# xuekt98/BBDM

Hardware: NVIDIA H100
Metric: denoising-steps/sec (UNet fwd) at 256^2 pixel-BBDM (higher is better)
Workload: dtype bf16x3 (split-bf16 tensor-core products, fp32 accumulate: fp32-class)

## Files before the change

bbdm_b200/cabi.py:

```python
from __future__ import annotations

import ctypes as C
import gc
import os

import torch

_HERE = os.path.dirname(os.path.abspath(__file__))
LIB_PATH = os.environ.get("BBDM_LIB") or os.path.join(_HERE, "libbbdm_b200.so")

ABI_VERSION = 7
OBJ = {"grad": 0, "noise": 1, "ysubx": 2}
RESAMPLE_NONE, RESAMPLE_UP2, RESAMPLE_DOWN2 = 0, 1, 2
RES_NONE, RES_SAME, RES_UP2, RES_DOWN2 = 0, 1, 2, 3
GN_MAX_SLICES = 64
ATTN_HEAD_DIMS = (16, 32, 64, 128)
ATTN_TC_HEAD_DIMS = (64, 128)
LN_MAX_C = 2048


def layernorm_bwd_workspace(rows, C):
    return -(-rows // 64) * 2 * C

SYMBOLS = [
    "bbdm_abi_version", "bbdm_last_error", "bbdm_device_info", "bbdm_check_device_fault",
    "bbdm_bridge_q_sample", "bbdm_bridge_p_sample", "bbdm_bridge_p_sample_dev", "bbdm_nchw_to_nhwc_cat", "bbdm_nhwc_to_nchw",
    "bbdm_gather_rows", "bbdm_linear_f32", "bbdm_gn_stats", "bbdm_prep_operand",
    "bbdm_pack_weight_split", "bbdm_pack_weight_split_padded", "bbdm_pack_weight_split_taps", "bbdm_pack_weight_split_dgrad",
    "bbdm_pack_weight_f32", "bbdm_conv_umma", "bbdm_conv_direct",
    "bbdm_attention", "bbdm_attention_split", "bbdm_attention_tc", "bbdm_conv_umma_geometry", "bbdm_gn_finalize_partials",
    "bbdm_split_grad", "bbdm_conv_wgrad_workspace", "bbdm_conv_wgrad", "bbdm_gn_bwd_reduce", "bbdm_gn_bwd_apply",
    "bbdm_conv_wgrad_direct", "bbdm_attention_bwd", "bbdm_conv_direct_pad", "bbdm_softmax_rows_split", "bbdm_vq_nearest", "bbdm_s2d_split", "bbdm_pack_weight_split_both",
    "bbdm_wino_geometry", "bbdm_wino_input", "bbdm_wino_output", "bbdm_wino_pack_weight",
    "bbdm_wino6_geometry", "bbdm_wino6_input", "bbdm_wino6_output", "bbdm_wino6_pack_weight",
    "bbdm_optim_chunk_elems", "bbdm_adam_multi", "bbdm_ema_multi", "bbdm_denorm_to_uint8",
    "bbdm_layernorm_split", "bbdm_geglu_split", "bbdm_attention_cross", "bbdm_conv_stem", "bbdm_spatial_rescale",
    "bbdm_layernorm_bwd", "bbdm_geglu_bwd", "bbdm_attention_cross_bwd",
]


class PSampleCoef(C.Structure):
    _fields_ = [("m_t", C.c_float), ("one_minus_m_t", C.c_float), ("sqrt_var_t", C.c_float),
                ("m_nt", C.c_float), ("one_minus_m_nt", C.c_float), ("c_xt", C.c_float),
                ("sigma_t", C.c_float)]


class PrepArgs(C.Structure):
    _fields_ = [("src1", C.c_void_p), ("c1", C.c_int), ("src2", C.c_void_p), ("c2", C.c_int),
                ("B", C.c_int), ("Hs", C.c_int), ("Ws", C.c_int), ("groups", C.c_int),
                ("mean", C.c_void_p), ("rstd", C.c_void_p), ("gamma", C.c_void_p), ("beta", C.c_void_p),
                ("film_scale", C.c_void_p), ("film_shift", C.c_void_p), ("film_stride", C.c_int64),
                ("silu", C.c_int), ("resample", C.c_int),
                ("act_f32", C.c_void_p), ("act_hi", C.c_void_p), ("act_lo", C.c_void_p),
                ("raw_f32", C.c_void_p), ("raw_hi", C.c_void_p), ("raw_lo", C.c_void_p)]


class ConvArgs(C.Structure):
    _fields_ = [("B", C.c_int), ("H", C.c_int), ("W", C.c_int),
                ("Cin", C.c_int), ("Cout", C.c_int), ("taps", C.c_int),
                ("a_hi", C.c_void_p), ("a_lo", C.c_void_p), ("w_hi", C.c_void_p), ("w_lo", C.c_void_p),
                ("bias", C.c_void_p),
                ("Cin2", C.c_int),
                ("a2_hi", C.c_void_p), ("a2_lo", C.c_void_p), ("w2_hi", C.c_void_p), ("w2_lo", C.c_void_p),
                ("bias2", C.c_void_p),
                ("residual", C.c_void_p), ("res_mode", C.c_int),
                ("out", C.c_void_p), ("out_hi", C.c_void_p), ("out_lo", C.c_void_p),
                ("passes", C.c_int), ("out_nchw_channels", C.c_int), ("upsample2x", C.c_int),
                ("stats_partial", C.c_void_p), ("weights_per_image", C.c_int), ("operand_f16", C.c_int),
                ("window_origin", C.c_int)]


class WinoInputArgs(C.Structure):
    _fields_ = [("src1", C.c_void_p), ("c1", C.c_int), ("src2", C.c_void_p), ("c2", C.c_int),
                ("B", C.c_int), ("H", C.c_int), ("W", C.c_int), ("groups", C.c_int),
                ("mean", C.c_void_p), ("rstd", C.c_void_p), ("gamma", C.c_void_p), ("beta", C.c_void_p),
                ("film_scale", C.c_void_p), ("film_shift", C.c_void_p), ("film_stride", C.c_int64),
                ("silu", C.c_int),
                ("v_hi", C.c_void_p), ("v_lo", C.c_void_p), ("raw_hi", C.c_void_p), ("raw_lo", C.c_void_p),
                ("act_hi", C.c_void_p), ("act_lo", C.c_void_p), ("down2", C.c_int)]


class WinoOutputArgs(C.Structure):
    _fields_ = [("m", C.c_void_p), ("inv_wscale", C.c_void_p), ("B", C.c_int), ("H", C.c_int), ("W", C.c_int), ("Cout", C.c_int),
                ("bias", C.c_void_p), ("residual", C.c_void_p), ("res_mode", C.c_int),
                ("out", C.c_void_p), ("stats_partial", C.c_void_p), ("up2_phases", C.c_int)]


class BbdmError(RuntimeError):
    pass


_lib = None


def load():
    global _lib
    if _lib is not None:
        return _lib
    if not os.path.exists(LIB_PATH):
        raise BbdmError(
            f"{LIB_PATH} not found: build the sm_90a kernels first (python -m bbdm_b200.build). "
            "bbdm_b200 has no PyTorch/CPU fallback for its kernels.")
    lib = C.CDLL(LIB_PATH)
    vp, i, i64, f = C.c_void_p, C.c_int, C.c_int64, C.c_float
    lib.bbdm_abi_version.restype = i
    lib.bbdm_last_error.restype = C.c_char_p
    lib.bbdm_device_info.argtypes = [C.POINTER(i)] * 3
    lib.bbdm_check_device_fault.argtypes = [vp, C.POINTER(C.c_ulonglong)]
    lib.bbdm_bridge_q_sample.argtypes = [vp, vp, vp, vp, vp, vp, i, i, vp, vp, i, i64, vp]
    lib.bbdm_bridge_p_sample.argtypes = [vp, vp, vp, vp, PSampleCoef, i, i, i, vp, vp, i64, vp]
    lib.bbdm_bridge_p_sample_dev.argtypes = [vp, vp, vp, vp, vp, i, i, i, vp, vp, i64, vp]
    lib.bbdm_nchw_to_nhwc_cat.argtypes = [vp, i, vp, i, i, i, i, vp, vp]
    lib.bbdm_nhwc_to_nchw.argtypes = [vp, i, i, i, i, vp, vp]
    lib.bbdm_gather_rows.argtypes = [vp, i, i, vp, i, vp, vp]
    lib.bbdm_linear_f32.argtypes = [vp, vp, vp, vp, i, i, i, i, i, vp]
    lib.bbdm_gn_stats.argtypes = [vp, i, vp, i, i, i, i, i, f, vp, vp, vp, vp]
    lib.bbdm_prep_operand.argtypes = [C.POINTER(PrepArgs), vp]
    lib.bbdm_pack_weight_split.argtypes = [vp, i, i, i, vp, vp, vp]
    lib.bbdm_pack_weight_split_padded.argtypes = [vp, i, i, i, i, vp, vp, vp]
    lib.bbdm_pack_weight_split_dgrad.argtypes = [vp, i, i, i, vp, vp, vp]
    lib.bbdm_pack_weight_split_taps.argtypes = [vp, i, i, i, vp, vp, vp]
    lib.bbdm_pack_weight_f32.argtypes = [vp, i, i, i, vp, vp]
    lib.bbdm_conv_umma.argtypes = [C.POINTER(ConvArgs), vp]
    lib.bbdm_conv_direct.argtypes = [vp, vp, vp, vp, vp, i, i, i, i, i, i, i, vp]
    lib.bbdm_conv_stem.argtypes = [vp, vp, vp, vp, i, i, i, i, i, vp, vp]
    lib.bbdm_attention.argtypes = [vp, i, i, i, i, i, vp, vp, vp, vp]
    lib.bbdm_conv_umma_geometry.argtypes = [i, i, C.POINTER(i), C.POINTER(i), C.POINTER(i), C.POINTER(i)]
    lib.bbdm_gn_finalize_partials.argtypes = [vp, i, i, vp, i, i, i, i, i, f, vp, vp, vp]
    lib.bbdm_split_grad.argtypes = [vp, i64, i, vp, vp, vp, vp, i64, vp, vp, vp]
    lib.bbdm_conv_wgrad_workspace.argtypes = [i, i, i, i, i, i, C.POINTER(i), C.POINTER(i64)]
    lib.bbdm_conv_wgrad.argtypes = [vp, vp, i64, vp, vp, i, i, i, i, i, i, i, vp, vp, vp]
    lib.bbdm_conv_wgrad_direct.argtypes = [vp, vp, i, i, i, i, i, i, vp, vp, i64, vp]
    lib.bbdm_gn_bwd_reduce.argtypes = [vp, vp, i, i, i, i, i, vp, vp, vp, vp, vp, vp, i64, i, vp, vp, vp]
    lib.bbdm_gn_bwd_apply.argtypes = [vp, vp, i, i, i, i, i, vp, vp, vp, vp, vp, vp, i64, i, vp, vp, vp, vp]
    lib.bbdm_attention_split.argtypes = [vp, vp, i, i, i, i, i, vp, vp, vp, vp]
    lib.bbdm_attention_tc.argtypes = [vp, vp, i, i, i, i, i, vp, vp, vp, vp]
    lib.bbdm_attention_bwd.argtypes = [vp, vp, vp, i, i, i, i, i, vp, vp, vp, vp]
    lib.bbdm_conv_direct_pad.argtypes = [vp, vp, vp, vp, vp, i, i, i, i, i, i, i, i, i, vp]
    lib.bbdm_softmax_rows_split.argtypes = [vp, i64, i64, C.c_float, vp, vp, vp]
    lib.bbdm_vq_nearest.argtypes = [vp, vp, i64, i, i, vp, vp, vp]
    lib.bbdm_s2d_split.argtypes = [vp, i, i, i, i, vp, vp, vp]
    lib.bbdm_pack_weight_split_both.argtypes = [vp, i, i, i, vp, vp, vp, vp, vp]
    lib.bbdm_wino_geometry.argtypes = [i, i, i, C.POINTER(i), C.POINTER(i), C.POINTER(i64), C.POINTER(i)]
    lib.bbdm_wino_input.argtypes = [C.POINTER(WinoInputArgs), vp]
    lib.bbdm_wino_output.argtypes = [C.POINTER(WinoOutputArgs), vp]
    lib.bbdm_wino_pack_weight.argtypes = [vp, i, i, i, vp, vp, vp, vp]
    lib.bbdm_wino6_geometry.argtypes = lib.bbdm_wino_geometry.argtypes
    lib.bbdm_wino6_input.argtypes = lib.bbdm_wino_input.argtypes
    lib.bbdm_wino6_output.argtypes = lib.bbdm_wino_output.argtypes
    lib.bbdm_wino6_pack_weight.argtypes = lib.bbdm_wino_pack_weight.argtypes
    lib.bbdm_denorm_to_uint8.argtypes = [vp, i, i, i, i, i, vp, vp]
    lib.bbdm_spatial_rescale.argtypes = [vp, i, i, i, i, i, vp, vp, i, vp, vp]
    lib.bbdm_layernorm_split.argtypes = [vp, i64, i, vp, vp, f, vp, vp, vp, vp]
    lib.bbdm_geglu_split.argtypes = [vp, i64, i, vp, vp, vp, vp]
    lib.bbdm_attention_cross.argtypes = [vp, vp, vp, vp, i, i, i, i, i, vp, vp, vp, vp]
    lib.bbdm_layernorm_bwd.argtypes = [vp, vp, i64, i, vp, f, vp, vp, vp, vp, vp]
    lib.bbdm_geglu_bwd.argtypes = [vp, vp, i64, i, vp, vp]
    lib.bbdm_attention_cross_bwd.argtypes = [vp, vp, vp, vp, i, i, i, i, i, vp, vp, vp, vp, vp]
    lib.bbdm_optim_chunk_elems.argtypes = []
    lib.bbdm_adam_multi.argtypes = [vp, vp, vp, vp, vp, vp, i, vp, vp, C.c_double, C.c_double, C.c_double, C.c_double,
                                     C.c_double, i64, vp, C.c_double, vp]
    lib.bbdm_ema_multi.argtypes = [vp, vp, vp, vp, vp, i, vp, C.c_double, i, vp]
    for s in SYMBOLS:
        fn = getattr(lib, s)
        if s not in ("bbdm_last_error",):
            fn.restype = i
    if lib.bbdm_abi_version() != ABI_VERSION:
        raise BbdmError(f"libbbdm_b200.so ABI {lib.bbdm_abi_version()} != binding ABI {ABI_VERSION}")
    _lib = lib
    return lib


def check(rc: int):
    if rc != 0:
        raise BbdmError(f"bbdm_b200 C-ABI call failed ({rc}): {load().bbdm_last_error().decode()}")


def ptr(t):
    return None if t is None else t.data_ptr()


def stream():
    return torch.cuda.current_stream().cuda_stream


def _device_guarded(fn):
    import functools

    @functools.wraps(fn)
    def wrapper(self, *args, **kw):
        dev = None
        for a in args:
            if isinstance(a, torch.Tensor) and a.is_cuda:
                dev = a.device.index
                break
        if dev is None:
            for a in kw.values():
                if isinstance(a, torch.Tensor) and a.is_cuda:
                    dev = a.device.index
                    break
        if dev is None or dev == torch.cuda.current_device():
            return fn(self, *args, **kw)
        with torch.cuda.device(dev):
            return fn(self, *args, **kw)
    return wrapper


def _guard_all(cls):
    for name, fn in list(vars(cls).items()):
        if callable(fn) and not name.startswith("_") and name not in ("empty", "conv_geometry", "wgrad_workspace", "wino_geometry", "optim_chunk_elems"):
            setattr(cls, name, _device_guarded(fn))
    return cls


LAUNCHES = {"n": 0}


def _req(t, dtype=torch.float32):
    assert t.is_cuda and t.is_contiguous() and t.dtype == dtype, (t.device, t.dtype, t.is_contiguous())
    return t


def _pitch(hi_t, lo_t, rows, cols):
    assert hi_t.is_cuda and tuple(hi_t.shape) == (rows, cols) and hi_t.stride(1) == 1, (hi_t.shape, hi_t.stride())
    assert lo_t.shape == hi_t.shape and lo_t.stride() == hi_t.stride(), (hi_t.stride(), lo_t.stride())
    return hi_t.stride(0)


@_guard_all
class CudaBackend:

    name = "sm_90a"
    requires_cuda = True
    wino_tensor_scale = True
    wino_tiles = (4, 6)
    window_origin = True

    def __init__(self):
        self.lib = load()

    def empty(self, shape, dtype, device):
        try:
            return torch.empty(shape, dtype=dtype, device=device)
        except torch.OutOfMemoryError:
            gc.collect()
            return torch.empty(shape, dtype=dtype, device=device)

    def q_sample(self, x0, y, noise, t, m_t, var_t, objective, xt_out, obj_out):
        B = x0.shape[0]
        n = x0.numel() // B
        for z in (x0, y, noise, m_t, var_t, xt_out, obj_out):
            _req(z)
        _req(t, torch.int64)
        check(self.lib.bbdm_bridge_q_sample(ptr(x0), ptr(y), ptr(noise), ptr(t), ptr(m_t), ptr(var_t),
                                            m_t.numel(), OBJ[objective], ptr(xt_out), ptr(obj_out), B, n,
                                            stream()))
        LAUNCHES["n"] += 1

    def p_sample(self, x_t, y, eps, noise, coef, objective, clip, is_last, x_out, x0_out):
        for z in (x_t, y, eps, x_out):
            _req(z)
        c = PSampleCoef(*[float(v) for v in coef])
        check(self.lib.bbdm_bridge_p_sample(ptr(x_t), ptr(y), ptr(eps), ptr(noise), c, OBJ[objective],
                                            int(clip), int(is_last), ptr(x_out), ptr(x0_out), x_t.numel(),
                                            stream()))
        LAUNCHES["n"] += 1

    def p_sample_dev(self, x_t, y, eps, noise, coef_dev, objective, clip, is_last, x_out, x0_out):
        for z in (x_t, y, eps, x_out, coef_dev):
            _req(z)
        check(self.lib.bbdm_bridge_p_sample_dev(ptr(x_t), ptr(y), ptr(eps), ptr(noise), ptr(coef_dev),
                                                OBJ[objective], int(clip), int(is_last), ptr(x_out), ptr(x0_out),
                                                x_t.numel(), stream()))
        LAUNCHES["n"] += 1

    def nchw_to_nhwc_cat(self, x, ctx, out):
        B, c1, H, W = x.shape
        c2 = 0 if ctx is None else ctx.shape[1]
        check(self.lib.bbdm_nchw_to_nhwc_cat(ptr(_req(x)), c1, ptr(ctx), c2, B, H, W, ptr(_req(out)), stream()))
        LAUNCHES["n"] += 1

    def nhwc_to_nchw(self, src, out):
        B, H, W, Cc = src.shape
        check(self.lib.bbdm_nhwc_to_nchw(ptr(_req(src)), B, H, W, Cc, ptr(_req(out)), stream()))
        LAUNCHES["n"] += 1

    def gather_rows(self, table, idx, out):
        check(self.lib.bbdm_gather_rows(ptr(_req(table)), table.shape[0], table.shape[1],
                                        ptr(_req(idx, torch.int64)), idx.numel(), ptr(_req(out)), stream()))
        LAUNCHES["n"] += 1

    def linear(self, x, w, bias, out, act_in=False, act_out=False):
        B, K = x.shape
        N = w.shape[0]
        check(self.lib.bbdm_linear_f32(ptr(_req(x)), ptr(_req(w)), ptr(bias), ptr(_req(out)), B, K, N,
                                       int(act_in), int(act_out), stream()))
        LAUNCHES["n"] += (B + 7) // 8

    def gn_stats(self, src1, src2, groups, eps, mean, rstd, workspace):
        B, H, W, c1 = src1.shape
        c2 = 0 if src2 is None else src2.shape[3]
        check(self.lib.bbdm_gn_stats(ptr(_req(src1)), c1, ptr(src2), c2, B, H, W, groups, eps,
                                     ptr(_req(mean)), ptr(_req(rstd)), ptr(workspace), stream()))
        LAUNCHES["n"] += 2

    def prep(self, src1, src2, *, groups=32, mean=None, rstd=None, gamma=None, beta=None,
             film_scale=None, film_shift=None, film_stride=0, silu=True, resample=RESAMPLE_NONE,
             act_f32=None, act_hi=None, act_lo=None, raw_f32=None, raw_hi=None, raw_lo=None):
        B, Hs, Ws, c1 = src1.shape
        a = PrepArgs(ptr(_req(src1)), c1, ptr(src2), 0 if src2 is None else src2.shape[3], B, Hs, Ws, groups,
                     ptr(mean), ptr(rstd), ptr(gamma), ptr(beta), ptr(film_scale), ptr(film_shift),
                     film_stride, int(silu), resample, ptr(act_f32), ptr(act_hi), ptr(act_lo),
                     ptr(raw_f32), ptr(raw_hi), ptr(raw_lo))
        check(self.lib.bbdm_prep_operand(C.byref(a), stream()))
        LAUNCHES["n"] += 1

    def pack_weight_split(self, w, hi, lo):
        Cout, Cin, k = w.shape[0], w.shape[1], (w.shape[2] if w.dim() > 2 else 1)
        check(self.lib.bbdm_pack_weight_split_padded(ptr(_req(w)), Cout, Cin, k, hi.shape[1], ptr(hi), ptr(lo),
                                                     stream()))
        LAUNCHES["n"] += 1

    def pack_weight_split_dgrad(self, w, hi, lo):
        Cout, Cin, k = w.shape[0], w.shape[1], w.shape[2]
        check(self.lib.bbdm_pack_weight_split_dgrad(ptr(_req(w)), Cout, Cin, k, ptr(hi), ptr(lo), stream()))
        LAUNCHES["n"] += 1

    def pack_weight_split_both(self, w, f_hi, f_lo, d_hi=None, d_lo=None):
        Cout, Cin, k = w.shape[0], w.shape[1], w.shape[2]
        check(self.lib.bbdm_pack_weight_split_both(ptr(_req(w)), Cout, Cin, k, ptr(f_hi), ptr(f_lo), ptr(d_hi), ptr(d_lo),
                                                   stream()))
        LAUNCHES["n"] += 1

    def pack_weight_split_taps(self, w, hi, lo):
        Cout, Cin, taps = w.shape
        check(self.lib.bbdm_pack_weight_split_taps(ptr(_req(w)), Cout, Cin, taps, ptr(hi), ptr(lo), stream()))
        LAUNCHES["n"] += 1

    def pack_weight_f32(self, w, out):
        Cout, Cin, k = w.shape[0], w.shape[1], (w.shape[2] if w.dim() > 2 else 1)
        check(self.lib.bbdm_pack_weight_f32(ptr(_req(w)), Cout, Cin, k, ptr(_req(out)), stream()))
        LAUNCHES["n"] += 1

    def conv_umma(self, *, B, H, W, Cin, Cout, taps, a_hi, a_lo, w_hi, w_lo, bias=None, Cin2=0,
                  a2_hi=None, a2_lo=None, w2_hi=None, w2_lo=None, bias2=None, residual=None,
                  res_mode=RES_NONE, out=None, out_hi=None, out_lo=None, passes=3, out_nchw_channels=0,
                  stats_partial=None, upsample2x=False, weights_per_image=False, operand_f16=False, window_origin=0):
        a = ConvArgs(B, H, W, Cin, Cout, taps, ptr(a_hi), ptr(a_lo), ptr(w_hi), ptr(w_lo), ptr(bias),
                     Cin2, ptr(a2_hi), ptr(a2_lo), ptr(w2_hi), ptr(w2_lo), ptr(bias2),
                     ptr(residual), res_mode, ptr(out), ptr(out_hi), ptr(out_lo), passes, out_nchw_channels,
                     int(upsample2x), ptr(stats_partial), int(weights_per_image), int(operand_f16), int(window_origin))
        check(self.lib.bbdm_conv_umma(C.byref(a), stream()))
        LAUNCHES["n"] += 1

    def conv_geometry(self, H, W):
        v = [C.c_int(0) for _ in range(4)]
        check(self.lib.bbdm_conv_umma_geometry(H, W, *[C.byref(z) for z in v]))
        return tuple(z.value for z in v)

    def _wino(self, name, tile):
        assert tile in self.wino_tiles, tile
        return getattr(self.lib, f"bbdm_wino{'' if tile == 4 else tile}_{name}")

    def wino_geometry(self, B, H, W, tile=4):
        th, tw, el, tot = C.c_int(0), C.c_int(0), C.c_int(0), C.c_int64(0)
        check(self._wino("geometry", tile)(B, H, W, C.byref(th), C.byref(tw), C.byref(tot), C.byref(el)))
        return th.value, tw.value, tot.value, bool(el.value)

    def wino_input(self, src1, src2, *, groups=32, mean=None, rstd=None, gamma=None, beta=None, film_scale=None,
                   film_shift=None, film_stride=0, silu=True, v_hi, v_lo, raw_hi=None, raw_lo=None, act_hi=None,
                   act_lo=None, tile=4, down2=False):
        B, H, W, c1 = src1.shape
        a = WinoInputArgs(ptr(_req(src1)), c1, ptr(src2), 0 if src2 is None else src2.shape[3], B, H, W, groups,
                          ptr(mean), ptr(rstd), ptr(gamma), ptr(beta), ptr(film_scale), ptr(film_shift), film_stride,
                          int(silu), ptr(_req(v_hi, torch.float16)), ptr(_req(v_lo, torch.float16)),
                          ptr(raw_hi), ptr(raw_lo), ptr(act_hi), ptr(act_lo), int(down2))
        check(self._wino("input", tile)(C.byref(a), stream()))
        LAUNCHES["n"] += 1

    def wino_output(self, m, *, B, H, W, Cout, bias=None, residual=None, res_mode=RES_NONE, out, stats_partial=None,
                    inv_wscale=None, tile=4, up2_phases=False):
        a = WinoOutputArgs(ptr(_req(m)), None if inv_wscale is None else ptr(_req(inv_wscale)), B, H, W, Cout, ptr(bias), ptr(residual), res_mode, ptr(_req(out)),
                           ptr(stats_partial), int(up2_phases))
        check(self._wino("output", tile)(C.byref(a), stream()))
        LAUNCHES["n"] += 1

    def wino_pack_weight(self, w, u_hi, u_lo, dgrad=False, inv_wscale=None, tile=4):
        Cout, Cin = w.shape[0], w.shape[1]
        check(self._wino("pack_weight", tile)(ptr(_req(w)), Cout, Cin, int(dgrad), ptr(_req(u_hi, torch.float16)),
                                              ptr(_req(u_lo, torch.float16)),
                                              None if inv_wscale is None else ptr(_req(inv_wscale)), stream()))
        LAUNCHES["n"] += 1

    def layernorm_split(self, x, gamma, beta, eps, out_f32=None, out_hi=None, out_lo=None):
        Cc = x.shape[-1]
        check(self.lib.bbdm_layernorm_split(ptr(_req(x)), x.numel() // Cc, Cc, ptr(_req(gamma)), ptr(_req(beta)), eps,
                                            ptr(out_f32), ptr(out_hi), ptr(out_lo), stream()))
        LAUNCHES["n"] += 1

    def geglu_split(self, u, out_f32=None, out_hi=None, out_lo=None):
        N2 = u.shape[-1]
        check(self.lib.bbdm_geglu_split(ptr(_req(u)), u.numel() // N2, N2 // 2, ptr(out_f32), ptr(out_hi), ptr(out_lo),
                                        stream()))
        LAUNCHES["n"] += 1

    def attention_cross(self, q_hi, q_lo, kv_hi, kv_lo, heads, out_f32=None, out_hi=None, out_lo=None):
        B, Tq, Cc = q_hi.shape
        Tkv = kv_hi.shape[1]
        check(self.lib.bbdm_attention_cross(ptr(_req(q_hi, torch.bfloat16)), ptr(_req(q_lo, torch.bfloat16)),
                                            ptr(_req(kv_hi, torch.bfloat16)), ptr(_req(kv_lo, torch.bfloat16)), B, Tq, Tkv,
                                            Cc, heads, ptr(out_f32), ptr(out_hi), ptr(out_lo), stream()))
        LAUNCHES["n"] += 1

    def layernorm_bwd(self, x, dy, gamma, eps, dx, dgamma, dbeta, workspace):
        Cc = x.shape[-1]
        check(self.lib.bbdm_layernorm_bwd(ptr(_req(x)), ptr(_req(dy)), x.numel() // Cc, Cc, ptr(_req(gamma)), eps,
                                          ptr(_req(dx)), ptr(_req(dgamma)), ptr(_req(dbeta)), ptr(_req(workspace)),
                                          stream()))
        LAUNCHES["n"] += 2

    def geglu_bwd(self, u, dy, du):
        N2 = u.shape[-1]
        check(self.lib.bbdm_geglu_bwd(ptr(_req(u)), ptr(_req(dy)), u.numel() // N2, N2 // 2, ptr(_req(du)), stream()))
        LAUNCHES["n"] += 1

    def attention_cross_bwd(self, q, kv, out, dout, heads, dq, dkv, lse, delta):
        B, Tq, Cc = q.shape
        check(self.lib.bbdm_attention_cross_bwd(ptr(_req(q)), ptr(_req(kv)), ptr(_req(out)), ptr(_req(dout)), B, Tq,
                                                kv.shape[1], Cc, heads, ptr(_req(dq)), ptr(_req(dkv)), ptr(_req(lse)),
                                                ptr(_req(delta)), stream()))
        LAUNCHES["n"] += 2

    def denorm_to_uint8(self, images, to_normal, out):
        B, Cc, H, W = images.shape
        check(self.lib.bbdm_denorm_to_uint8(ptr(_req(images)), B, Cc, H, W, int(to_normal), ptr(_req(out, torch.uint8)),
                                            stream()))
        LAUNCHES["n"] += 1

    def spatial_rescale(self, src, n_stages, weight, bias, out):
        B, Cc, H, W = src.shape
        cout = 0 if weight is None else int(weight.shape[0])
        check(self.lib.bbdm_spatial_rescale(ptr(_req(src)), B, Cc, H, W, int(n_stages),
                                            ptr(None if weight is None else _req(weight)),
                                            ptr(None if bias is None else _req(bias)), cout, ptr(_req(out)), stream()))
        LAUNCHES["n"] += 1

    def optim_chunk_elems(self):
        return int(self.lib.bbdm_optim_chunk_elems())

    def adam_multi(self, tab, exp_avg, exp_avg_sq, *, lr, beta1, beta2, eps, weight_decay, step, ema_shadow=None,
                   ema_decay=0.0):
        check(self.lib.bbdm_adam_multi(ptr(tab.params), ptr(tab.grads), ptr(tab.numel), ptr(tab.offsets),
                                       ptr(tab.chunk_tensor), ptr(tab.chunk_index), tab.n_chunks, ptr(_req(exp_avg)),
                                       ptr(_req(exp_avg_sq)), lr, beta1, beta2, eps, weight_decay, int(step),
                                       ptr(ema_shadow), float(ema_decay), stream()))
        LAUNCHES["n"] += 1

    def ema_multi(self, tab, shadow, decay, with_decay=True):
        check(self.lib.bbdm_ema_multi(ptr(tab.params), ptr(tab.numel), ptr(tab.offsets), ptr(tab.chunk_tensor),
                                      ptr(tab.chunk_index), tab.n_chunks, ptr(_req(shadow)), float(decay), int(with_decay),
                                      stream()))
        LAUNCHES["n"] += 1

    def gn_finalize_partials(self, part1, rows1, part2, rows2, B, hw, groups, eps, mean, rstd):
        c1 = part1.shape[1]
        c2 = 0 if part2 is None else part2.shape[1]
        check(self.lib.bbdm_gn_finalize_partials(ptr(_req(part1)), c1, rows1, ptr(part2), c2, rows2, B, hw, groups,
                                                 eps, ptr(_req(mean)), ptr(_req(rstd)), stream()))
        LAUNCHES["n"] += 1

    def split_grad(self, src, hi, lo, hi_t, lo_t, colsum=None, workspace=None):
        P, Cc = src.numel() // src.shape[-1], src.shape[-1]
        ld = _pitch(hi_t, lo_t, Cc, P)
        check(self.lib.bbdm_split_grad(ptr(_req(src)), P, Cc, ptr(hi), ptr(lo), ptr(hi_t), ptr(lo_t), ld, ptr(colsum),
                                       ptr(workspace), stream()))
        LAUNCHES["n"] += 1 + (colsum is not None)

    def wgrad_workspace(self, B, H, W, Cin, Cout, taps):
        sp, fl = C.c_int(0), C.c_int64(0)
        check(self.lib.bbdm_conv_wgrad_workspace(B, H, W, Cin, Cout, taps, C.byref(sp), C.byref(fl)))
        return sp.value, fl.value

    def conv_wgrad(self, g_hi_t, g_lo_t, a_hi, a_lo, B, H, W, Cin, Cout, taps, dw, workspace, window_origin=0):
        ld = _pitch(g_hi_t, g_lo_t, Cout, B * H * W)
        check(self.lib.bbdm_conv_wgrad(ptr(g_hi_t), ptr(g_lo_t), ld, ptr(a_hi), ptr(a_lo), B, H, W, Cin, Cout, taps,
                                       int(window_origin), ptr(_req(dw)), ptr(_req(workspace)), stream()))
        LAUNCHES["n"] += 2

    def conv_wgrad_direct(self, dy, x, k, dw, workspace):
        B, H, W, Cin = x.shape
        Cout = dy.shape[3]
        check(self.lib.bbdm_conv_wgrad_direct(ptr(_req(dy)), ptr(_req(x)), B, H, W, Cin, Cout, k, ptr(_req(dw)),
                                              ptr(_req(workspace)), workspace.numel(), stream()))
        LAUNCHES["n"] += 2

    def gn_bwd_reduce(self, x, da, groups, mean, rstd, gamma, beta, fscale, fshift, fstride, silu, a12, ws):
        B, H, W, Cc = x.shape
        check(self.lib.bbdm_gn_bwd_reduce(ptr(_req(x)), ptr(_req(da)), B, H, W, Cc, groups, ptr(mean), ptr(rstd),
                                          ptr(gamma), ptr(beta), ptr(fscale), ptr(fshift), fstride, int(silu),
                                          ptr(_req(a12)), ptr(_req(ws)), stream()))
        LAUNCHES["n"] += 2

    def gn_bwd_apply(self, x, da, groups, mean, rstd, gamma, beta, fscale, fshift, fstride, silu, s1, s2, dx):
        B, H, W, Cc = x.shape
        check(self.lib.bbdm_gn_bwd_apply(ptr(_req(x)), ptr(_req(da)), B, H, W, Cc, groups, ptr(mean), ptr(rstd),
                                         ptr(gamma), ptr(beta), ptr(fscale), ptr(fshift), fstride, int(silu),
                                         ptr(_req(s1)), ptr(_req(s2)), ptr(_req(dx)), stream()))
        LAUNCHES["n"] += 1

    def conv_direct(self, src, w_packed, bias, residual, out, Cout, k, stride=1):
        B, H, W, Cin = src.shape
        check(self.lib.bbdm_conv_direct(ptr(_req(src)), ptr(_req(w_packed)), ptr(bias), ptr(residual),
                                        ptr(_req(out)), B, H, W, Cin, Cout, k, stride, stream()))
        LAUNCHES["n"] += 1

    def conv_stem(self, src, w_packed, bias, out, Cout, stats_partial=None):
        B, H, W, Cin = src.shape
        check(self.lib.bbdm_conv_stem(ptr(_req(src)), ptr(_req(w_packed)), ptr(bias), ptr(_req(out)), B, H, W, Cin, Cout,
                                      ptr(stats_partial), stream()))
        LAUNCHES["n"] += 1

    def attention(self, qkv, heads, order, out_f32=None, out_hi=None, out_lo=None):
        B, T, C3 = qkv.shape
        check(self.lib.bbdm_attention(ptr(_req(qkv)), B, T, C3 // 3, heads, order, ptr(out_f32),
                                      ptr(out_hi), ptr(out_lo), stream()))
        LAUNCHES["n"] += 1

    def attention_split(self, qkv_hi, qkv_lo, heads, order, out_f32=None, out_hi=None, out_lo=None):
        B, T, C3 = qkv_hi.shape
        check(self.lib.bbdm_attention_split(ptr(_req(qkv_hi, torch.bfloat16)), ptr(_req(qkv_lo, torch.bfloat16)),
                                            B, T, C3 // 3, heads, order, ptr(out_f32), ptr(out_hi), ptr(out_lo),
                                            stream()))
        LAUNCHES["n"] += 1

    def attention_tc(self, qkv_hi, qkv_lo, heads, order, out_f32=None, out_hi=None, out_lo=None):
        B, T, C3 = qkv_hi.shape
        check(self.lib.bbdm_attention_tc(ptr(_req(qkv_hi, torch.bfloat16)), ptr(_req(qkv_lo, torch.bfloat16)),
                                         B, T, C3 // 3, heads, order, ptr(out_f32), ptr(out_hi), ptr(out_lo), stream()))
        LAUNCHES["n"] += 1

    def attention_bwd(self, qkv, out, dout, heads, order, dqkv, lse, delta):
        B, T, C3 = qkv.shape
        check(self.lib.bbdm_attention_bwd(ptr(_req(qkv)), ptr(_req(out)), ptr(_req(dout)), B, T, C3 // 3, heads, order,
                                          ptr(_req(dqkv)), ptr(_req(lse)), ptr(_req(delta)), stream()))
        LAUNCHES["n"] += 2

    def conv_direct_pad(self, src, w_packed, bias, residual, out, cout, k, stride, pad_lo, pad_hi):
        B, H, W, Cin = src.shape
        check(self.lib.bbdm_conv_direct_pad(ptr(_req(src)), ptr(_req(w_packed)), ptr(bias), ptr(residual), ptr(_req(out)),
                                            B, H, W, Cin, cout, k, stride, pad_lo, pad_hi, stream()))
        LAUNCHES["n"] += 1

    def softmax_rows_split(self, src, scale, out_hi, out_lo):
        rows, cols = src.numel() // src.shape[-1], src.shape[-1]
        check(self.lib.bbdm_softmax_rows_split(ptr(_req(src)), rows, cols, float(scale), ptr(_req(out_hi, torch.bfloat16)),
                                               ptr(_req(out_lo, torch.bfloat16)), stream()))
        LAUNCHES["n"] += 1

    def s2d_split(self, src, out_hi, out_lo):
        B, H, W, Cc = src.shape
        check(self.lib.bbdm_s2d_split(ptr(_req(src)), B, H, W, Cc, ptr(_req(out_hi, torch.bfloat16)),
                                      ptr(_req(out_lo, torch.bfloat16)), stream()))
        LAUNCHES["n"] += 1

    def vq_nearest(self, z, codebook, z_q, indices):
        n, d = z.numel() // z.shape[-1], z.shape[-1]
        check(self.lib.bbdm_vq_nearest(ptr(_req(z)), ptr(_req(codebook)), n, codebook.shape[0], d, ptr(_req(z_q)),
                                       ptr(_req(indices, torch.int64)), stream()))
        LAUNCHES["n"] += 1

    def check_fault(self, device=None):
        w = C.c_ulonglong(0)
        if device is not None and torch.device(device).index not in (None, torch.cuda.current_device()):
            with torch.cuda.device(device):
                check(self.lib.bbdm_check_device_fault(stream(), C.byref(w)))
            return
        check(self.lib.bbdm_check_device_fault(stream(), C.byref(w)))
```

bbdm_b200/csrc/conv_umma.cu:

```cuda
#include "tc_common.cuh"
#include <stdlib.h>

namespace bbdm {

constexpr int UM_BM = 128;
constexpr int UM_BK = 64;
constexpr int UM_THREADS = 384;
constexpr int UM_PRODUCER_REGS = 40, UM_CONSUMER_REGS = 232;
static_assert(128 * UM_PRODUCER_REGS + 256 * UM_CONSUMER_REGS <= 65536, "conv_umma: register split");
constexpr int UM_SLICES = 4;

struct ConvParams {
  int B, H, W, Cout;
  int TW, TH, TB, tiles_w, tiles_h, tiles_b, n_tiles;
  int kb_per_tap;
  int K1;
  int K2;
  int taps;
  int up2;
  int origin;
  int w_per_image;
  int kb_per_chunk;
  const float* bias; const float* bias2;
  const float* residual; int res_mode;
  float* out; __nv_bfloat16* out_hi; __nv_bfloat16* out_lo;
  int out_nchw_c;
  float* stats;
  unsigned long long* fault;
};

template <int BN>
struct UmmaCfg {
  static constexpr uint32_t A_BYTES = UM_BM * UM_BK * 2;
  static constexpr uint32_t W_BYTES = BN * UM_BK * 2;
  static constexpr uint32_t STAGE3 = 2 * A_BYTES + 2 * W_BYTES;
  static constexpr uint32_t STAGE1 = A_BYTES + W_BYTES;
  static constexpr uint32_t SMEM_BUDGET = 200 * 1024;
  static constexpr int STAGES3 = (SMEM_BUDGET / STAGE3) > 6 ? 6 : (SMEM_BUDGET / STAGE3);
  static constexpr int STAGES1 = (SMEM_BUDGET / STAGE1) > 8 ? 8 : (SMEM_BUDGET / STAGE1);
};

template <int BN, bool F16>
__device__ __forceinline__ void conv_mma(float* d, uint64_t da, uint64_t db) {
  if (F16) {
    if (BN == 128) wgmma_n128_f16<0>(d, da, db, 1u); else wgmma_n64_f16<0>(d, da, db, 1u);
  } else {
    if (BN == 128) wgmma_n128_bf16<0>(d, da, db, 1u); else wgmma_n64_bf16<0>(d, da, db, 1u);
  }
}

struct EpiTile {
  int nb, tw, th, tb, phase;
  int bb[2], hh[2], ww[2];
  bool valid[2];
  int64_t pix[2];
};

__device__ __forceinline__ EpiTile epi_tile(const ConvParams& p, int tile, int n_blocks, int warp, int lane) {
  EpiTile e;
  e.nb = tile % n_blocks;
  int mt = tile / n_blocks;
  e.phase = 0;
  if (p.up2) { e.phase = mt & 3; mt >>= 2; }
  e.tw = mt % p.tiles_w; mt /= p.tiles_w;
  e.th = mt % p.tiles_h;
  e.tb = mt / p.tiles_h;
  const int OH = p.up2 ? 2 * p.H : p.H, OW = p.up2 ? 2 * p.W : p.W;
#pragma unroll
  for (int ri = 0; ri < 2; ++ri) {
    const int row = 16 * warp + (lane >> 2) + 8 * ri;
    const int ws = e.tw * p.TW + row % p.TW;
    const int hs = e.th * p.TH + (row / p.TW) % p.TH;
    e.bb[ri] = e.tb * p.TB + row / (p.TW * p.TH);
    e.valid[ri] = ws < p.W && hs < p.H && e.bb[ri] < p.B;
    e.hh[ri] = p.up2 ? 2 * hs + (e.phase >> 1) : hs;
    e.ww[ri] = p.up2 ? 2 * ws + (e.phase & 1) : ws;
    e.pix[ri] = ((int64_t)e.bb[ri] * OH + e.hh[ri]) * OW + e.ww[ri];
  }
  return e;
}

template <int BN>
__device__ __forceinline__ void epi_slice(const ConvParams& p, const float* racc, EpiTile e, int s, int warp,
                                          int lane, float (*stats_s)[BN][2]) {
  constexpr int JS = BN / 8 / UM_SLICES;
  asm volatile("" : "+r"(e.nb), "+r"(e.bb[0]), "+r"(e.bb[1]), "+r"(e.hh[0]), "+r"(e.hh[1]), "+r"(e.ww[0]),
               "+r"(e.ww[1]), "+l"(e.pix[0]), "+l"(e.pix[1]));
  const int OH = p.up2 ? 2 * p.H : p.H, OW = p.up2 ? 2 * p.W : p.W;
  const int n0 = e.nb * BN + 2 * (lane & 3);
  float2 v[2][JS];
#pragma unroll
  for (int ri = 0; ri < 2; ++ri) {
#pragma unroll
    for (int j = 0; j < JS; ++j) {
      const int jj = JS * s + j;
      const int nc = n0 + 8 * jj;
      v[ri][j] = make_float2(racc[4 * jj + 2 * ri], racc[4 * jj + 2 * ri + 1]);
      if (p.bias) { const float2 b = *reinterpret_cast<const float2*>(p.bias + nc); v[ri][j].x += b.x; v[ri][j].y += b.y; }
      if (p.bias2) { const float2 b = *reinterpret_cast<const float2*>(p.bias2 + nc); v[ri][j].x += b.x; v[ri][j].y += b.y; }
    }
  }
  if (p.res_mode == BBDM_RES_SAME || p.res_mode == BBDM_RES_UP2) {
#pragma unroll
    for (int ri = 0; ri < 2; ++ri) {
      if (!e.valid[ri]) continue;
      const int64_t rpix = p.res_mode == BBDM_RES_SAME
                               ? e.pix[ri]
                               : ((int64_t)e.bb[ri] * (OH >> 1) + (e.hh[ri] >> 1)) * (OW >> 1) + (e.ww[ri] >> 1);
      const float* rp = p.residual + rpix * p.Cout + n0 + 8 * JS * s;
#pragma unroll
      for (int j = 0; j < JS; ++j) {
        const float2 t = *reinterpret_cast<const float2*>(rp + 8 * j);
        v[ri][j].x += t.x; v[ri][j].y += t.y;
      }
    }
  } else if (p.res_mode == BBDM_RES_DOWN2) {
    const int64_t W2 = (int64_t)OW * 2;
#pragma unroll
    for (int ri = 0; ri < 2; ++ri) {
      if (!e.valid[ri]) continue;
      const float* rp0 = p.residual + (((int64_t)e.bb[ri] * OH * 2 + e.hh[ri] * 2) * W2 + e.ww[ri] * 2) * p.Cout +
                         n0 + 8 * JS * s;
#pragma unroll
      for (int j = 0; j < JS; ++j) {
        const float* rp = rp0 + 8 * j;
        const float2 t0 = *reinterpret_cast<const float2*>(rp), t1 = *reinterpret_cast<const float2*>(rp + p.Cout);
        const float2 t2 = *reinterpret_cast<const float2*>(rp + W2 * p.Cout);
        const float2 t3 = *reinterpret_cast<const float2*>(rp + (W2 + 1) * p.Cout);
        v[ri][j].x += 0.25f * (((t0.x + t1.x) + t2.x) + t3.x);
        v[ri][j].y += 0.25f * (((t0.y + t1.y) + t2.y) + t3.y);
      }
    }
  }
  float ssum[2 * JS], ssq[2 * JS];
#pragma unroll
  for (int j = 0; j < 2 * JS; ++j) { ssum[j] = 0.f; ssq[j] = 0.f; }
#pragma unroll
  for (int ri = 0; ri < 2; ++ri) {
    if (!e.valid[ri]) continue;
    const int bb = e.bb[ri], hh = e.hh[ri], ww = e.ww[ri];
    const int64_t pix = e.pix[ri];
#pragma unroll
    for (int j = 0; j < JS; ++j) {
      const int nc = n0 + 8 * (JS * s + j);
      const float2 w = v[ri][j];
      if (p.out_nchw_c > 0) {
        if (nc < p.out_nchw_c) p.out[(((int64_t)bb * p.out_nchw_c + nc) * OH + hh) * OW + ww] = w.x;
        if (nc + 1 < p.out_nchw_c) p.out[(((int64_t)bb * p.out_nchw_c + nc + 1) * OH + hh) * OW + ww] = w.y;
      } else if (p.out) {
        *reinterpret_cast<float2*>(p.out + pix * p.Cout + nc) = w;
      }
      if (p.out_hi) {
        uint32_t h, l;
        split2x(w.x, w.y, h, l);
        *reinterpret_cast<uint32_t*>(p.out_hi + pix * p.Cout + nc) = h;
        *reinterpret_cast<uint32_t*>(p.out_lo + pix * p.Cout + nc) = l;
      }
      ssum[2 * j] += w.x; ssq[2 * j] += w.x * w.x;
      ssum[2 * j + 1] += w.y; ssq[2 * j + 1] += w.y * w.y;
    }
  }
  if (p.stats) {
#pragma unroll
    for (int j = 0; j < 2 * JS; ++j) {
#pragma unroll
      for (int off = 4; off < 32; off <<= 1) {
        ssum[j] += __shfl_xor_sync(0xffffffffu, ssum[j], off);
        ssq[j] += __shfl_xor_sync(0xffffffffu, ssq[j], off);
      }
    }
    if (lane < 4) {
#pragma unroll
      for (int j = 0; j < 2 * JS; ++j) {
        const int c = 8 * (JS * s + (j >> 1)) + 2 * lane + (j & 1);
        stats_s[warp][c][0] = ssum[j];
        stats_s[warp][c][1] = ssq[j];
      }
    }
  }
}

template <int BN>
__device__ __forceinline__ void epi_stats_out(const ConvParams& p, const EpiTile& e, float (*stats_s)[BN][2]) {
  if (!p.stats) return;
  asm volatile("bar.sync 1, 256;" ::: "memory");
  const int64_t tile_lin =
      (((int64_t)e.tb * p.tiles_w * p.tiles_h + e.th * p.tiles_w + e.tw) * (p.up2 ? 4 : 1) + e.phase) * 4;
  int i0 = threadIdx.x;
  asm volatile("" : "+r"(i0));
  for (int i = i0; i < 4 * BN; i += 256) {
    const int q = i / BN, c = i % BN;
    const float s = stats_s[2 * q][c][0] + stats_s[2 * q + 1][c][0];
    const float sq = stats_s[2 * q][c][1] + stats_s[2 * q + 1][c][1];
    *reinterpret_cast<float2*>(p.stats + ((tile_lin + q) * p.Cout + e.nb * BN + c) * 2) = make_float2(s, sq);
  }
  asm volatile("bar.sync 1, 256;" ::: "memory");
}

template <int BN>
__device__ __forceinline__ void epi_slices(const ConvParams& p, const float* racc, const EpiTile& e, int s_begin,
                                           int s_end, int warp, int lane, float (*stats_s)[BN][2]) {
#pragma unroll
  for (int s = 0; s < UM_SLICES; ++s)
    if (s >= s_begin && s < s_end) epi_slice<BN>(p, racc, e, s, warp, lane, stats_s);
}

template <int BN, int PASSES, bool F16>
__global__ void __launch_bounds__(UM_THREADS, 1)
conv_umma_kernel(const __grid_constant__ CUtensorMap map_a_hi, const __grid_constant__ CUtensorMap map_a_lo,
                 const __grid_constant__ CUtensorMap map_w_hi, const __grid_constant__ CUtensorMap map_w_lo,
                 const __grid_constant__ CUtensorMap map_a2_hi, const __grid_constant__ CUtensorMap map_a2_lo,
                 const __grid_constant__ CUtensorMap map_w2_hi, const __grid_constant__ CUtensorMap map_w2_lo,
                 const ConvParams p) {
  using Cfg = UmmaCfg<BN>;
  constexpr int STAGES = PASSES == 3 ? Cfg::STAGES3 : Cfg::STAGES1;
  constexpr uint32_t STAGE_BYTES = PASSES == 3 ? Cfg::STAGE3 : Cfg::STAGE1;
  constexpr uint32_t OFF_ALO = Cfg::A_BYTES;
  constexpr uint32_t OFF_WHI = PASSES == 3 ? 2 * Cfg::A_BYTES : Cfg::A_BYTES;
  constexpr uint32_t OFF_WLO = OFF_WHI + Cfg::W_BYTES;
  constexpr int NR = BN / 2;
  static_assert(STAGES >= 2, "need at least a double buffer");

  extern __shared__ uint8_t smem_raw[];
  __shared__ __align__(8) uint64_t bars[2 * 8];
  __shared__ int abort_s;
  __shared__ __align__(16) float stats_s[8][BN][2];

  const uint32_t tiles_base = (smem_u32(smem_raw) + 1023u) & ~1023u;
  const int warp = threadIdx.x >> 5, lane = threadIdx.x & 31;
  const uint32_t bar_full = smem_u32(&bars[0]);
  const uint32_t bar_empty = smem_u32(&bars[8]);
  volatile int* abort_flag = &abort_s;

  if (threadIdx.x == 0) {
    abort_s = 0;
    for (int i = 0; i < STAGES; ++i) { mbar_init(bar_full + 8 * i, 1); mbar_init(bar_empty + 8 * i, 8); }
    asm volatile("fence.mbarrier_init.release.cluster;" ::: "memory");
  }
  __syncthreads();

  const int n_blocks = p.Cout / BN;
  const int total_tiles = p.n_tiles * n_blocks * (p.up2 ? 4 : 1);
  const int KB = p.K1 + p.K2;

  if (warp >= 8) {
    setmaxnreg_dec<UM_PRODUCER_REGS>();
    if (warp == 8 && lane == 0) {
      int stage = 0;
      uint32_t phase_bit = 0;
      for (int tile = blockIdx.x; tile < total_tiles; tile += gridDim.x) {
        const int nb = tile % n_blocks;
        int mt = tile / n_blocks;
        int phase = 0;
        if (p.up2) { phase = mt & 3; mt >>= 2; }
        const int tw = mt % p.tiles_w; mt /= p.tiles_w;
        const int th = mt % p.tiles_h;
        const int tb = mt / p.tiles_h;
        const int w0 = tw * p.TW, h0 = th * p.TH, b0 = tb * p.TB, n0 = nb * BN;
        for (int kb = 0; kb < KB; ++kb) {
          mbar_wait(bar_empty + 8 * stage, phase_bit ^ 1, abort_flag, p.fault, 0xE0000000ull | (unsigned)kb);
          const uint32_t sbase = tiles_base + stage * STAGE_BYTES;
          const uint32_t full = bar_full + 8 * stage;
          mbar_expect_tx(full, STAGE_BYTES);
          if (kb < p.K1) {
            const int tap = kb / p.kb_per_tap, cb = kb - tap * p.kb_per_tap;
            int dy = 0, dx = 0, wtap = tap;
            if (p.up2) {
              const int r = tap >> 1, c = tap & 1;
              dy = (phase >> 1) ? r : r - 1;
              dx = (phase & 1) ? c : c - 1;
              wtap = phase * 4 + tap;
            } else if (p.taps == 9) { dy = tap / 3 - 1; dx = tap % 3 - 1; }
            else if (p.taps == 4) { dy = (tap >> 1) + p.origin; dx = (tap & 1) + p.origin; }
            else if (p.w_per_image) wtap = tb;
            tma_load_4d(sbase, &map_a_hi, full, cb * UM_BK, w0 + dx, h0 + dy, b0);
            if (PASSES == 3) tma_load_4d(sbase + OFF_ALO, &map_a_lo, full, cb * UM_BK, w0 + dx, h0 + dy, b0);
            tma_load_3d(sbase + OFF_WHI, &map_w_hi, full, cb * UM_BK, n0, wtap);
            if (PASSES == 3) tma_load_3d(sbase + OFF_WLO, &map_w_lo, full, cb * UM_BK, n0, wtap);
          } else {
            const int cb = kb - p.K1;
            tma_load_4d(sbase, &map_a2_hi, full, cb * UM_BK, w0, h0, b0);
            if (PASSES == 3) tma_load_4d(sbase + OFF_ALO, &map_a2_lo, full, cb * UM_BK, w0, h0, b0);
            tma_load_3d(sbase + OFF_WHI, &map_w2_hi, full, cb * UM_BK, n0, 0);
            if (PASSES == 3) tma_load_3d(sbase + OFF_WLO, &map_w2_lo, full, cb * UM_BK, n0, 0);
          }
          if (++stage == STAGES) { stage = 0; phase_bit ^= 1; }
        }
      }
    }
    return;
  }

  setmaxnreg_inc<UM_CONSUMER_REGS>();
  const int wg = warp >> 2;
  const uint32_t a_off = (uint32_t)wg * 64 * 128;
  int stage = 0;
  uint32_t phase_bit = 0;
  float racc[NR];
  EpiTile pend;
  bool pending = false;
  int slice = 0;
  for (int tile = blockIdx.x; tile < total_tiles; tile += gridDim.x) {
    for (int kb0 = 0; kb0 < KB; kb0 += p.kb_per_chunk) {
      const int kb1 = kb0 + p.kb_per_chunk < KB ? kb0 + p.kb_per_chunk : KB;
      float acc[NR];
#pragma unroll
      for (int j = 0; j < NR; ++j) acc[j] = 0.f;
      int prev = -1;
      for (int kb = kb0; kb < kb1; ++kb) {
        mbar_wait(bar_full + 8 * stage, phase_bit, abort_flag, p.fault, 0xF0000000ull | (unsigned)kb);
        const uint32_t sbase = tiles_base + stage * STAGE_BYTES;
        const uint64_t da_hi = make_sw128_desc(sbase + a_off);
        const uint64_t da_lo = make_sw128_desc(sbase + OFF_ALO + a_off);
        const uint64_t db_hi = make_sw128_desc(sbase + OFF_WHI);
        const uint64_t db_lo = make_sw128_desc(sbase + OFF_WLO);
        wgmma_fence();
#pragma unroll
        for (int k = 0; k < UM_BK / 16; ++k) {
          const uint64_t ko = (uint64_t)(k * 32 >> 4);
          if (PASSES == 3) {
            conv_mma<BN, F16>(acc, da_lo + ko, db_hi + ko);
            conv_mma<BN, F16>(acc, da_hi + ko, db_lo + ko);
          }
          conv_mma<BN, F16>(acc, da_hi + ko, db_hi + ko);
        }
        wgmma_commit();
        wgmma_wait<1>();
        if (prev >= 0 && lane == 0) mbar_arrive(bar_empty + 8 * prev);
        prev = stage;
        if (++stage == STAGES) { stage = 0; phase_bit ^= 1; }
        if (pending) {
          const int s_end = kb + 1 < kb1 ? slice + 1 : UM_SLICES;
          epi_slices<BN>(p, racc, pend, slice, s_end, warp, lane, stats_s);
          slice = s_end;
        }
      }
      if (pending) {
        epi_stats_out<BN>(p, pend, stats_s);
        pending = false;
      }
      wgmma_wait<0>();
      reg_fence<NR>(acc);
      if (lane == 0) mbar_arrive(bar_empty + 8 * prev);
      if (kb0 == 0) {
#pragma unroll
        for (int j = 0; j < NR; ++j) racc[j] = 0.f + acc[j];
      } else {
#pragma unroll
        for (int j = 0; j < NR; ++j) racc[j] += acc[j];
      }
    }
    pend = epi_tile(p, tile, n_blocks, warp, lane);
    pending = true;
    slice = 0;
  }
  if (pending) {
    epi_slices<BN>(p, racc, pend, 0, UM_SLICES, warp, lane, stats_s);
    epi_stats_out<BN>(p, pend, stats_s);
  }
}

static int make_act_map(CUtensorMap* m, const void* ptr, int B, int H, int W, int C, int TW, int TH, int TB,
                        bool f16) {
  EncodeTiledFn enc = get_encode();
  BBDM_REQUIRE(enc != nullptr, "cuTensorMapEncodeTiled entry point not available");
  cuuint64_t dims[4] = {(cuuint64_t)C, (cuuint64_t)W, (cuuint64_t)H, (cuuint64_t)B};
  cuuint64_t strides[3] = {(cuuint64_t)C * 2, (cuuint64_t)W * C * 2, (cuuint64_t)H * W * C * 2};
  cuuint32_t box[4] = {(cuuint32_t)UM_BK, (cuuint32_t)TW, (cuuint32_t)TH, (cuuint32_t)TB};
  cuuint32_t es[4] = {1, 1, 1, 1};
  CUresult r = enc(m, f16 ? CU_TENSOR_MAP_DATA_TYPE_FLOAT16 : CU_TENSOR_MAP_DATA_TYPE_BFLOAT16, 4, const_cast<void*>(ptr), dims, strides, box, es,
                   CU_TENSOR_MAP_INTERLEAVE_NONE, CU_TENSOR_MAP_SWIZZLE_128B, CU_TENSOR_MAP_L2_PROMOTION_L2_256B,
                   CU_TENSOR_MAP_FLOAT_OOB_FILL_NONE);
  BBDM_REQUIRE(r == CUDA_SUCCESS, "cuTensorMapEncodeTiled(activation) failed: %d (B=%d H=%d W=%d C=%d box=%dx%dx%d)",
               (int)r, B, H, W, C, TW, TH, TB);
  return BBDM_OK;
}

static int make_w_map(CUtensorMap* m, const void* ptr, int taps, int Cout, int Cin, int BN, bool f16) {
  EncodeTiledFn enc = get_encode();
  BBDM_REQUIRE(enc != nullptr, "cuTensorMapEncodeTiled entry point not available");
  cuuint64_t dims[3] = {(cuuint64_t)Cin, (cuuint64_t)Cout, (cuuint64_t)taps};
  cuuint64_t strides[2] = {(cuuint64_t)Cin * 2, (cuuint64_t)Cout * Cin * 2};
  cuuint32_t box[3] = {(cuuint32_t)UM_BK, (cuuint32_t)BN, 1};
  cuuint32_t es[3] = {1, 1, 1};
  CUresult r = enc(m, f16 ? CU_TENSOR_MAP_DATA_TYPE_FLOAT16 : CU_TENSOR_MAP_DATA_TYPE_BFLOAT16, 3, const_cast<void*>(ptr), dims, strides, box, es,
                   CU_TENSOR_MAP_INTERLEAVE_NONE, CU_TENSOR_MAP_SWIZZLE_128B, CU_TENSOR_MAP_L2_PROMOTION_L2_256B,
                   CU_TENSOR_MAP_FLOAT_OOB_FILL_NONE);
  BBDM_REQUIRE(r == CUDA_SUCCESS, "cuTensorMapEncodeTiled(weight) failed: %d (taps=%d Cout=%d Cin=%d BN=%d)", (int)r,
               taps, Cout, Cin, BN);
  return BBDM_OK;
}

static int pow2_floor(int x) { int p = 1; while (p * 2 <= x) p *= 2; return p; }
static int pow2_ceil(int x) { int p = 1; while (p < x) p *= 2; return p; }

template <int BN, int PASSES, bool F16>
static int launch_conv(const CUtensorMap* maps, const ConvParams& p, int grid, cudaStream_t s) {
  using Cfg = UmmaCfg<BN>;
  constexpr int STAGES = PASSES == 3 ? Cfg::STAGES3 : Cfg::STAGES1;
  constexpr uint32_t STAGE_BYTES = PASSES == 3 ? Cfg::STAGE3 : Cfg::STAGE1;
  const size_t smem = (size_t)STAGES * STAGE_BYTES + 1024;
  static DeviceOnce configured;
  if (configured.need()) {
    BBDM_CUDA_CHECK(cudaFuncSetAttribute(conv_umma_kernel<BN, PASSES, F16>, cudaFuncAttributeMaxDynamicSharedMemorySize, (int)smem));
    configured.mark();
  }
  conv_umma_kernel<BN, PASSES, F16><<<grid, UM_THREADS, smem, s>>>(maps[0], maps[1], maps[2], maps[3], maps[4], maps[5],
                                                                  maps[6], maps[7], p);
  BBDM_LAUNCH_CHECK();
  return BBDM_OK;
}

}

using namespace bbdm;

static void tile_geometry(int H, int W, int* TW, int* TH, int* TB) {
  *TW = pow2_floor(W) < 16 ? pow2_floor(W) : 16;
  const int th = pow2_ceil(H);
  *TH = th < UM_BM / *TW ? th : UM_BM / *TW;
  *TB = UM_BM / (*TW * *TH);
}

extern "C" int bbdm_conv_umma_geometry(int H, int W, int* TW, int* TH, int* TB, int* rows_per_image) {
  BBDM_REQUIRE(H > 0 && W >= 4, "conv_umma_geometry: need H > 0, W >= 4");
  int tw, th, tb;
  tile_geometry(H, W, &tw, &th, &tb);
  if (TW) *TW = tw;
  if (TH) *TH = th;
  if (TB) *TB = tb;
  if (rows_per_image) *rows_per_image = tb == 1 ? 4 * ((W + tw - 1) / tw) * ((H + th - 1) / th) : 0;
  return BBDM_OK;
}

extern "C" int bbdm_conv_umma(const BbdmConvArgs* a, void* stream) {
  BBDM_REQUIRE(a != nullptr, "conv_umma: null args");
  BBDM_REQUIRE(a->B > 0 && a->H > 0 && a->W > 0, "conv_umma: bad spatial shape");
  BBDM_REQUIRE(a->taps == 1 || a->taps == 9 || a->taps == 4, "conv_umma: taps must be 1, 4 or 9 (got %d)", a->taps);
  BBDM_REQUIRE(!a->upsample2x || (a->taps == 4 && a->Cin2 == 0), "conv_umma: upsample2x needs the 16 phase taps and no fused 1x1");
  BBDM_REQUIRE(a->Cin > 0 && a->Cin % 64 == 0, "conv_umma: Cin %% 64 != 0 (Cin=%d)", a->Cin);
  BBDM_REQUIRE(a->Cout > 0 && a->Cout % 64 == 0, "conv_umma: Cout %% 64 != 0 (Cout=%d)", a->Cout);
  BBDM_REQUIRE(a->Cin2 >= 0 && a->Cin2 % 64 == 0, "conv_umma: Cin2 %% 64 != 0 (Cin2=%d)", a->Cin2);
  BBDM_REQUIRE(a->passes == 1 || a->passes == 3, "conv_umma: passes must be 1 or 3");
  BBDM_REQUIRE(a->a_hi && a->w_hi && (a->passes == 1 || (a->a_lo && a->w_lo)), "conv_umma: missing operand plane");
  if (a->Cin2) BBDM_REQUIRE(a->a2_hi && a->w2_hi && (a->passes == 1 || (a->a2_lo && a->w2_lo)), "conv_umma: missing 1x1 operand plane");
  BBDM_REQUIRE(a->out || (a->out_hi && a->out_lo), "conv_umma: no output");
  BBDM_REQUIRE((a->out_hi == nullptr) == (a->out_lo == nullptr), "conv_umma: out hi/lo must come in pairs");
  BBDM_REQUIRE(a->res_mode >= 0 && a->res_mode <= 3 && (a->res_mode == 0 || a->residual), "conv_umma: bad residual");
  if (a->res_mode == BBDM_RES_UP2 && !a->upsample2x) BBDM_REQUIRE(a->H % 2 == 0 && a->W % 2 == 0, "conv_umma: RES_UP2 needs even H, W");
  BBDM_REQUIRE(a->W >= 4, "conv_umma: W < 4 not supported (use conv_direct)");
  BBDM_REQUIRE(a->window_origin == 0 || a->window_origin == -1, "conv_umma: window_origin must be 0 or -1 (got %d)",
               a->window_origin);
  BBDM_REQUIRE(a->window_origin == 0 || (a->taps == 4 && !a->upsample2x),
               "conv_umma: window_origin -1 needs taps == 4 and no upsample2x");
  const bool wpi = a->weights_per_image != 0, f16 = a->operand_f16 != 0;
  if (wpi) BBDM_REQUIRE(a->taps == 1 && a->Cin2 == 0 && !a->upsample2x, "conv_umma: weights_per_image needs taps == 1 and no fused operand");

  ConvParams p;
  p.B = a->B; p.H = a->H; p.W = a->W; p.Cout = a->Cout;
  tile_geometry(a->H, a->W, &p.TW, &p.TH, &p.TB);
  p.tiles_w = (a->W + p.TW - 1) / p.TW;
  p.tiles_h = (a->H + p.TH - 1) / p.TH;
  p.tiles_b = (a->B + p.TB - 1) / p.TB;
  p.n_tiles = p.tiles_w * p.tiles_h * p.tiles_b;
  int BN = (a->Cout % 128 == 0) ? 128 : 64;
  {
    const int64_t m_tiles = (int64_t)p.n_tiles * (a->upsample2x ? 4 : 1);
    const int64_t want = (int64_t)(0.7 * num_sms());
    if (BN > 64 && m_tiles * (a->Cout / BN) < want) BN = 64;
  }
  p.kb_per_tap = a->Cin / UM_BK;
  p.K1 = a->taps * p.kb_per_tap;
  p.K2 = a->Cin2 / UM_BK;
  p.taps = a->taps;
  p.up2 = a->upsample2x ? 1 : 0;
  p.origin = a->window_origin;
  p.w_per_image = wpi ? 1 : 0;
  static int wino_chunk = -1;
  if (wino_chunk < 0) { const char* e = getenv("BBDM_WINO_CHUNK"); wino_chunk = (e && atoi(e) > 0) ? atoi(e) : 0; }
  const int wchunk = wino_chunk ? wino_chunk : (a->Cin >= 512 ? 4 : 2);
  p.kb_per_chunk = wpi ? wchunk : (a->passes == 3 ? 4 : 8);
  if (wpi) BBDM_REQUIRE(p.TB == 1, "conv_umma: weights_per_image needs 128-pixel tiles inside one image (H*W >= 128)");
  p.bias = a->bias; p.bias2 = a->Cin2 ? a->bias2 : nullptr;
  p.residual = a->residual; p.res_mode = a->res_mode;
  p.out = a->out; p.out_hi = (__nv_bfloat16*)a->out_hi; p.out_lo = (__nv_bfloat16*)a->out_lo;
  p.out_nchw_c = a->out_nchw_channels;
  p.stats = a->stats_partial;
  BBDM_REQUIRE(p.out_nchw_c >= 0 && p.out_nchw_c <= a->Cout && (p.out_nchw_c == 0 || (a->out && !a->out_hi)),
               "conv_umma: bad out_nchw_channels");
  p.fault = device_fault_ptr();
  BBDM_REQUIRE(p.fault != nullptr, "conv_umma: device fault word unavailable");

  BBDM_REQUIRE(p.stats == nullptr || (p.TB == 1 && p.out_nchw_c == 0),
               "conv_umma: stats_partial needs a tile inside one image (H*W >= 128) and NHWC output");
  CUtensorMap maps[8];
  int rc;
  if ((rc = make_act_map(&maps[0], a->a_hi, a->B, a->H, a->W, a->Cin, p.TW, p.TH, p.TB, f16))) return rc;
  if ((rc = make_act_map(&maps[1], a->passes == 3 ? a->a_lo : a->a_hi, a->B, a->H, a->W, a->Cin, p.TW, p.TH, p.TB, f16))) return rc;
  const int wtaps = a->upsample2x ? 16 : (wpi ? a->B : a->taps);
  if ((rc = make_w_map(&maps[2], a->w_hi, wtaps, a->Cout, a->Cin, BN, f16))) return rc;
  if ((rc = make_w_map(&maps[3], a->passes == 3 ? a->w_lo : a->w_hi, wtaps, a->Cout, a->Cin, BN, f16))) return rc;
  if (a->Cin2) {
    if ((rc = make_act_map(&maps[4], a->a2_hi, a->B, a->H, a->W, a->Cin2, p.TW, p.TH, p.TB, f16))) return rc;
    if ((rc = make_act_map(&maps[5], a->passes == 3 ? a->a2_lo : a->a2_hi, a->B, a->H, a->W, a->Cin2, p.TW, p.TH, p.TB, f16))) return rc;
    if ((rc = make_w_map(&maps[6], a->w2_hi, 1, a->Cout, a->Cin2, BN, f16))) return rc;
    if ((rc = make_w_map(&maps[7], a->passes == 3 ? a->w2_lo : a->w2_hi, 1, a->Cout, a->Cin2, BN, f16))) return rc;
  } else {
    maps[4] = maps[0]; maps[5] = maps[1]; maps[6] = maps[2]; maps[7] = maps[3];
  }
  const int64_t total = (int64_t)p.n_tiles * (a->Cout / BN) * (p.up2 ? 4 : 1);
  BBDM_REQUIRE(total < (1ll << 30), "conv_umma: too many tiles");
  const int grid = (int)(total < num_sms() ? total : num_sms());
  cudaStream_t s = (cudaStream_t)stream;
  const bool p3 = a->passes == 3;
  if (BN == 128) {
    if (f16) return p3 ? launch_conv<128, 3, true>(maps, p, grid, s) : launch_conv<128, 1, true>(maps, p, grid, s);
    return p3 ? launch_conv<128, 3, false>(maps, p, grid, s) : launch_conv<128, 1, false>(maps, p, grid, s);
  }
  if (f16) return p3 ? launch_conv<64, 3, true>(maps, p, grid, s) : launch_conv<64, 1, true>(maps, p, grid, s);
  return p3 ? launch_conv<64, 3, false>(maps, p, grid, s) : launch_conv<64, 1, false>(maps, p, grid, s);
}
```

bbdm_b200/csrc/tc_common.cuh:

```cuda
#pragma once
#include "common.cuh"
#include <cuda.h>

namespace bbdm {

__device__ __forceinline__ uint32_t smem_u32(const void* p) {
  return (uint32_t)__cvta_generic_to_shared(p);
}
__device__ __forceinline__ void mbar_init(uint32_t bar, uint32_t count) {
  asm volatile("mbarrier.init.shared::cta.b64 [%0], %1;" ::"r"(bar), "r"(count));
}
__device__ __forceinline__ void mbar_expect_tx(uint32_t bar, uint32_t bytes) {
  asm volatile("mbarrier.arrive.expect_tx.shared::cta.b64 _, [%0], %1;" ::"r"(bar), "r"(bytes) : "memory");
}
__device__ __forceinline__ void mbar_arrive(uint32_t bar) {
  asm volatile("mbarrier.arrive.shared::cta.b64 _, [%0];" ::"r"(bar) : "memory");
}
__device__ __forceinline__ bool mbar_try_wait(uint32_t bar, uint32_t parity) {
  uint32_t ok;
  asm volatile(
      "{\n\t.reg .pred P;\n\t"
      "mbarrier.try_wait.parity.shared::cta.b64 P, [%1], %2;\n\t"
      "selp.u32 %0, 1, 0, P;\n\t}"
      : "=r"(ok) : "r"(bar), "r"(parity) : "memory");
  return ok != 0;
}
__device__ __forceinline__ void mbar_wait(uint32_t bar, uint32_t parity, volatile int* abort_flag,
                                          unsigned long long* fault, unsigned long long code) {
  if (mbar_try_wait(bar, parity)) return;
  const long long t0 = clock64();
  while (!mbar_try_wait(bar, parity)) {
    if (*abort_flag) return;
    if (clock64() - t0 > 1000000000ll) {
      *abort_flag = 1;
      atomicExch(fault, code);
      return;
    }
  }
}
__device__ __forceinline__ void tma_load_4d(uint32_t dst, const CUtensorMap* map, uint32_t bar,
                                            int c0, int c1, int c2, int c3) {
  asm volatile(
      "cp.async.bulk.tensor.4d.shared::cluster.global.mbarrier::complete_tx::bytes"
      " [%0], [%1, {%3, %4, %5, %6}], [%2];"
      ::"r"(dst), "l"(map), "r"(bar), "r"(c0), "r"(c1), "r"(c2), "r"(c3) : "memory");
}
__device__ __forceinline__ void tma_load_4d_im2col(uint32_t dst, const CUtensorMap* map, uint32_t bar,
                                                   int c0, int w, int h, int n, uint16_t off_w, uint16_t off_h) {
  asm volatile(
      "cp.async.bulk.tensor.4d.shared::cluster.global.im2col.mbarrier::complete_tx::bytes"
      " [%0], [%1, {%3, %4, %5, %6}], [%2], {%7, %8};"
      ::"r"(dst), "l"(map), "r"(bar), "r"(c0), "r"(w), "r"(h), "r"(n), "h"(off_w), "h"(off_h) : "memory");
}
__device__ __forceinline__ void tma_load_2d(uint32_t dst, const CUtensorMap* map, uint32_t bar, int c0, int c1) {
  asm volatile(
      "cp.async.bulk.tensor.2d.shared::cluster.global.mbarrier::complete_tx::bytes"
      " [%0], [%1, {%3, %4}], [%2];"
      ::"r"(dst), "l"(map), "r"(bar), "r"(c0), "r"(c1) : "memory");
}
__device__ __forceinline__ void tma_load_3d(uint32_t dst, const CUtensorMap* map, uint32_t bar,
                                            int c0, int c1, int c2) {
  asm volatile(
      "cp.async.bulk.tensor.3d.shared::cluster.global.mbarrier::complete_tx::bytes"
      " [%0], [%1, {%3, %4, %5}], [%2];"
      ::"r"(dst), "l"(map), "r"(bar), "r"(c0), "r"(c1), "r"(c2) : "memory");
}
__device__ __forceinline__ void wgmma_fence() { asm volatile("wgmma.fence.sync.aligned;" ::: "memory"); }
__device__ __forceinline__ void wgmma_commit() { asm volatile("wgmma.commit_group.sync.aligned;" ::: "memory"); }
template <int N>
__device__ __forceinline__ void wgmma_wait() { asm volatile("wgmma.wait_group.sync.aligned %0;" ::"n"(N) : "memory"); }
template <int R>
__device__ __forceinline__ void reg_fence(float* d) {
#pragma unroll
  for (int i = 0; i < R; ++i) asm volatile("" : "+f"(d[i])::"memory");
}

__device__ __forceinline__ uint64_t make_sw128_desc(uint32_t saddr, uint32_t lbo = 16) {
  uint64_t d = 0;
  d |= (uint64_t)((saddr & 0x3FFFF) >> 4);
  d |= (uint64_t)((lbo & 0x3FFFF) >> 4) << 16;
  d |= (uint64_t)(1024 >> 4) << 32;
  d |= (uint64_t)1 << 62;
  return d;
}

template <int TB>
__device__ __forceinline__ void wgmma_n64_bf16(float* d, uint64_t da, uint64_t db, uint32_t scale_d) {
  asm volatile(
      "{\n\t.reg .pred p;\n\tsetp.ne.b32 p, %34, 0;\n\t"
      "wgmma.mma_async.sync.aligned.m64n64k16.f32.bf16.bf16 "
      "{%0, %1, %2, %3, %4, %5, %6, %7, %8, %9, %10, %11, %12, %13, %14, %15, %16, %17, %18, %19, %20, %21, %22, %23, %24, %25, %26, %27, %28, %29, %30, %31}, %32, %33, p, 1, 1, 0, %35;\n\t}"
      : "+f"(d[0]), "+f"(d[1]), "+f"(d[2]), "+f"(d[3]), "+f"(d[4]), "+f"(d[5]), "+f"(d[6]), "+f"(d[7]), "+f"(d[8]), "+f"(d[9]), "+f"(d[10]), "+f"(d[11]), "+f"(d[12]), "+f"(d[13]), "+f"(d[14]), "+f"(d[15]), "+f"(d[16]), "+f"(d[17]), "+f"(d[18]), "+f"(d[19]), "+f"(d[20]), "+f"(d[21]), "+f"(d[22]), "+f"(d[23]), "+f"(d[24]), "+f"(d[25]), "+f"(d[26]), "+f"(d[27]), "+f"(d[28]), "+f"(d[29]), "+f"(d[30]), "+f"(d[31])
      : "l"(da), "l"(db), "r"(scale_d), "n"(TB));
}
template <int TB>
__device__ __forceinline__ void wgmma_n64_f16(float* d, uint64_t da, uint64_t db, uint32_t scale_d) {
  asm volatile(
      "{\n\t.reg .pred p;\n\tsetp.ne.b32 p, %34, 0;\n\t"
      "wgmma.mma_async.sync.aligned.m64n64k16.f32.f16.f16 "
      "{%0, %1, %2, %3, %4, %5, %6, %7, %8, %9, %10, %11, %12, %13, %14, %15, %16, %17, %18, %19, %20, %21, %22, %23, %24, %25, %26, %27, %28, %29, %30, %31}, %32, %33, p, 1, 1, 0, %35;\n\t}"
      : "+f"(d[0]), "+f"(d[1]), "+f"(d[2]), "+f"(d[3]), "+f"(d[4]), "+f"(d[5]), "+f"(d[6]), "+f"(d[7]), "+f"(d[8]), "+f"(d[9]), "+f"(d[10]), "+f"(d[11]), "+f"(d[12]), "+f"(d[13]), "+f"(d[14]), "+f"(d[15]), "+f"(d[16]), "+f"(d[17]), "+f"(d[18]), "+f"(d[19]), "+f"(d[20]), "+f"(d[21]), "+f"(d[22]), "+f"(d[23]), "+f"(d[24]), "+f"(d[25]), "+f"(d[26]), "+f"(d[27]), "+f"(d[28]), "+f"(d[29]), "+f"(d[30]), "+f"(d[31])
      : "l"(da), "l"(db), "r"(scale_d), "n"(TB));
}
template <int TB>
__device__ __forceinline__ void wgmma_n128_bf16(float* d, uint64_t da, uint64_t db, uint32_t scale_d) {
  asm volatile(
      "{\n\t.reg .pred p;\n\tsetp.ne.b32 p, %66, 0;\n\t"
      "wgmma.mma_async.sync.aligned.m64n128k16.f32.bf16.bf16 "
      "{%0, %1, %2, %3, %4, %5, %6, %7, %8, %9, %10, %11, %12, %13, %14, %15, %16, %17, %18, %19, %20, %21, %22, %23, %24, %25, %26, %27, %28, %29, %30, %31, %32, %33, %34, %35, %36, %37, %38, %39, %40, %41, %42, %43, %44, %45, %46, %47, %48, %49, %50, %51, %52, %53, %54, %55, %56, %57, %58, %59, %60, %61, %62, %63}, %64, %65, p, 1, 1, 0, %67;\n\t}"
      : "+f"(d[0]), "+f"(d[1]), "+f"(d[2]), "+f"(d[3]), "+f"(d[4]), "+f"(d[5]), "+f"(d[6]), "+f"(d[7]), "+f"(d[8]), "+f"(d[9]), "+f"(d[10]), "+f"(d[11]), "+f"(d[12]), "+f"(d[13]), "+f"(d[14]), "+f"(d[15]), "+f"(d[16]), "+f"(d[17]), "+f"(d[18]), "+f"(d[19]), "+f"(d[20]), "+f"(d[21]), "+f"(d[22]), "+f"(d[23]), "+f"(d[24]), "+f"(d[25]), "+f"(d[26]), "+f"(d[27]), "+f"(d[28]), "+f"(d[29]), "+f"(d[30]), "+f"(d[31]), "+f"(d[32]), "+f"(d[33]), "+f"(d[34]), "+f"(d[35]), "+f"(d[36]), "+f"(d[37]), "+f"(d[38]), "+f"(d[39]), "+f"(d[40]), "+f"(d[41]), "+f"(d[42]), "+f"(d[43]), "+f"(d[44]), "+f"(d[45]), "+f"(d[46]), "+f"(d[47]), "+f"(d[48]), "+f"(d[49]), "+f"(d[50]), "+f"(d[51]), "+f"(d[52]), "+f"(d[53]), "+f"(d[54]), "+f"(d[55]), "+f"(d[56]), "+f"(d[57]), "+f"(d[58]), "+f"(d[59]), "+f"(d[60]), "+f"(d[61]), "+f"(d[62]), "+f"(d[63])
      : "l"(da), "l"(db), "r"(scale_d), "n"(TB));
}
template <int TB>
__device__ __forceinline__ void wgmma_n128_f16(float* d, uint64_t da, uint64_t db, uint32_t scale_d) {
  asm volatile(
      "{\n\t.reg .pred p;\n\tsetp.ne.b32 p, %66, 0;\n\t"
      "wgmma.mma_async.sync.aligned.m64n128k16.f32.f16.f16 "
      "{%0, %1, %2, %3, %4, %5, %6, %7, %8, %9, %10, %11, %12, %13, %14, %15, %16, %17, %18, %19, %20, %21, %22, %23, %24, %25, %26, %27, %28, %29, %30, %31, %32, %33, %34, %35, %36, %37, %38, %39, %40, %41, %42, %43, %44, %45, %46, %47, %48, %49, %50, %51, %52, %53, %54, %55, %56, %57, %58, %59, %60, %61, %62, %63}, %64, %65, p, 1, 1, 0, %67;\n\t}"
      : "+f"(d[0]), "+f"(d[1]), "+f"(d[2]), "+f"(d[3]), "+f"(d[4]), "+f"(d[5]), "+f"(d[6]), "+f"(d[7]), "+f"(d[8]), "+f"(d[9]), "+f"(d[10]), "+f"(d[11]), "+f"(d[12]), "+f"(d[13]), "+f"(d[14]), "+f"(d[15]), "+f"(d[16]), "+f"(d[17]), "+f"(d[18]), "+f"(d[19]), "+f"(d[20]), "+f"(d[21]), "+f"(d[22]), "+f"(d[23]), "+f"(d[24]), "+f"(d[25]), "+f"(d[26]), "+f"(d[27]), "+f"(d[28]), "+f"(d[29]), "+f"(d[30]), "+f"(d[31]), "+f"(d[32]), "+f"(d[33]), "+f"(d[34]), "+f"(d[35]), "+f"(d[36]), "+f"(d[37]), "+f"(d[38]), "+f"(d[39]), "+f"(d[40]), "+f"(d[41]), "+f"(d[42]), "+f"(d[43]), "+f"(d[44]), "+f"(d[45]), "+f"(d[46]), "+f"(d[47]), "+f"(d[48]), "+f"(d[49]), "+f"(d[50]), "+f"(d[51]), "+f"(d[52]), "+f"(d[53]), "+f"(d[54]), "+f"(d[55]), "+f"(d[56]), "+f"(d[57]), "+f"(d[58]), "+f"(d[59]), "+f"(d[60]), "+f"(d[61]), "+f"(d[62]), "+f"(d[63])
      : "l"(da), "l"(db), "r"(scale_d), "n"(TB));
}
template <int TB>
__device__ __forceinline__ void wgmma_rs_n64_bf16(float* d, const uint32_t* a, uint64_t db, uint32_t scale_d) {
  asm volatile(
      "{\n\t.reg .pred p;\n\tsetp.ne.b32 p, %37, 0;\n\t"
      "wgmma.mma_async.sync.aligned.m64n64k16.f32.bf16.bf16 "
      "{%0, %1, %2, %3, %4, %5, %6, %7, %8, %9, %10, %11, %12, %13, %14, %15, %16, %17, %18, %19, %20, %21, %22, %23, %24, %25, %26, %27, %28, %29, %30, %31}, {%32, %33, %34, %35}, %36, p, 1, 1, %38;\n\t}"
      : "+f"(d[0]), "+f"(d[1]), "+f"(d[2]), "+f"(d[3]), "+f"(d[4]), "+f"(d[5]), "+f"(d[6]), "+f"(d[7]), "+f"(d[8]), "+f"(d[9]), "+f"(d[10]), "+f"(d[11]), "+f"(d[12]), "+f"(d[13]), "+f"(d[14]), "+f"(d[15]), "+f"(d[16]), "+f"(d[17]), "+f"(d[18]), "+f"(d[19]), "+f"(d[20]), "+f"(d[21]), "+f"(d[22]), "+f"(d[23]), "+f"(d[24]), "+f"(d[25]), "+f"(d[26]), "+f"(d[27]), "+f"(d[28]), "+f"(d[29]), "+f"(d[30]), "+f"(d[31])
      : "r"(a[0]), "r"(a[1]), "r"(a[2]), "r"(a[3]), "l"(db), "r"(scale_d), "n"(TB));
}

template <int N>
__device__ __forceinline__ void setmaxnreg_inc() { asm volatile("setmaxnreg.inc.sync.aligned.u32 %0;" ::"n"(N)); }
template <int N>
__device__ __forceinline__ void setmaxnreg_dec() { asm volatile("setmaxnreg.dec.sync.aligned.u32 %0;" ::"n"(N)); }

__device__ __forceinline__ float ex2_approx(float x) {
  float y;
  asm("ex2.approx.ftz.f32 %0, %1;" : "=f"(y) : "f"(x));
  return y;
}
__device__ __forceinline__ void st_shared_v4(uint32_t addr, uint32_t a, uint32_t b, uint32_t c, uint32_t d) {
  asm volatile("st.shared.v4.b32 [%0], {%1, %2, %3, %4};" ::"r"(addr), "r"(a), "r"(b), "r"(c), "r"(d) : "memory");
}

typedef CUresult (*EncodeTiledFn)(CUtensorMap*, CUtensorMapDataType, cuuint32_t, void*, const cuuint64_t*,
                                  const cuuint64_t*, const cuuint32_t*, const cuuint32_t*, CUtensorMapInterleave,
                                  CUtensorMapSwizzle, CUtensorMapL2promotion, CUtensorMapFloatOOBfill);

static inline EncodeTiledFn get_encode() {
  static EncodeTiledFn fn = nullptr;
  if (!fn) {
    void* p = nullptr;
    cudaDriverEntryPointQueryResult qres;
    if (cudaGetDriverEntryPoint("cuTensorMapEncodeTiled", &p, cudaEnableDefault, &qres) == cudaSuccess &&
        qres == cudaDriverEntryPointSuccess)
      fn = (EncodeTiledFn)p;
  }
  return fn;
}

typedef CUresult (*EncodeIm2colFn)(CUtensorMap*, CUtensorMapDataType, cuuint32_t, void*, const cuuint64_t*,
                                   const cuuint64_t*, const int*, const int*, cuuint32_t, cuuint32_t, const cuuint32_t*,
                                   CUtensorMapInterleave, CUtensorMapSwizzle, CUtensorMapL2promotion,
                                   CUtensorMapFloatOOBfill);

static inline EncodeIm2colFn get_encode_im2col() {
  static EncodeIm2colFn fn = nullptr;
  if (!fn) {
    void* p = nullptr;
    cudaDriverEntryPointQueryResult qres;
    if (cudaGetDriverEntryPoint("cuTensorMapEncodeIm2col", &p, cudaEnableDefault, &qres) == cudaSuccess &&
        qres == cudaDriverEntryPointSuccess)
      fn = (EncodeIm2colFn)p;
  }
  return fn;
}

}
```

bbdm_b200/engine.py:

```python
from __future__ import annotations

import torch
import torch.nn as nn

from . import cabi, convs
from .transformer import SpatialTransformer
from .unet import (AttentionBlock, Downsample, ResBlock, TimestepEmbedSequential, UNetModel,
                   Upsample, timestep_embedding)

GN_GROUPS = 32
GN_EPS = 1e-5


def resample_to_res(resample):
    return {cabi.RESAMPLE_NONE: cabi.RES_SAME, cabi.RESAMPLE_UP2: cabi.RES_UP2,
            cabi.RESAMPLE_DOWN2: cabi.RES_DOWN2}[resample]


class _Pool:

    _serial = 0

    def __init__(self, backend, device):
        self.be, self.device, self.free = backend, device, {}
        self.bytes = 0
        _Pool._serial += 1
        self.serial = _Pool._serial

    def get(self, shape, dtype=torch.float32):
        key = (tuple(shape), dtype)
        lst = self.free.get(key)
        if lst:
            return lst.pop()
        t = self.be.empty(tuple(shape), dtype, self.device)
        self.bytes += t.numel() * t.element_size()
        return t

    def put(self, *ts):
        for t in ts:
            if t is not None:
                gn = t.__dict__.pop("_gn", None)
                if gn is not None:
                    self.put(gn[0])
                self.free.setdefault((tuple(t.shape), t.dtype), []).append(t)


class KernelExecutor:

    gn_eps = GN_EPS

    def __init__(self, backend=None, precision: str = "split3"):
        self.be = backend if backend is not None else cabi.CudaBackend()
        assert precision in ("split3", "bf16")
        self.passes = 3 if precision == "split3" else 1
        self.precision = precision
        self._pools = {}
        self._gn_ws = None
        self._geom_cache = {}
        self.wino = precision == "split3" and convs.WINOGRAD
        self.wino_min_c, self.wino_min_tiles = convs.WINO_MIN_C, convs.WINO_MIN_TILES
        self._wino_geom = {}

    def _umma_ok(self, cin, cout, w):
        return convs.tensor_core_ok(cin, cout, w)

    def _pool(self, device, shape_key=None):
        key = (device, shape_key)
        p = self._pools.pop(key, None)
        if p is None:
            p = _Pool(self.be, device)
            while len(self._pools) >= 2:
                self._pools.pop(next(iter(self._pools)))
        self._pools[key] = p
        return p

    def pool_serial(self, device, shape_key):
        return self._pool(device, shape_key).serial

    def pool_bytes(self):
        return sum(p.bytes for p in self._pools.values())

    def _stats(self, pool, src1, src2, eps=None):
        eps = self.gn_eps if eps is None else eps
        B = src1.shape[0]
        mean, rstd = pool.get((B, GN_GROUPS)), pool.get((B, GN_GROUPS))
        g1 = getattr(src1, "_gn", None)
        g2 = None if src2 is None else getattr(src2, "_gn", None)
        if g1 is not None and (src2 is None or g2 is not None):
            self.be.gn_finalize_partials(g1[0], g1[1], None if g2 is None else g2[0], 0 if g2 is None else g2[1],
                                         B, src1.shape[1] * src1.shape[2], GN_GROUPS, eps, mean, rstd)
            return mean, rstd
        if self._gn_ws is None or self._gn_ws.numel() < B * GN_GROUPS * cabi.GN_MAX_SLICES * 2 \
                or self._gn_ws.device != src1.device:
            self._gn_ws = self.be.empty((B * GN_GROUPS * cabi.GN_MAX_SLICES * 2,), torch.float64, src1.device)
        self.be.gn_stats(src1, src2, GN_GROUPS, eps, mean, rstd, self._gn_ws)
        return mean, rstd

    def _conv(self, pool, ent, *, a_f32=None, a_hi=None, a_lo=None, shape, bias=None, residual=None,
              res_mode=cabi.RES_NONE, second=None, out_split=False, want_f32=True, stride=1, out=None,
              stats=False, planes=None, taps=None, upsample2x=False, window_origin=0):
        B, H, W = shape
        bias = ent["bias"] if bias is None else bias
        if a_hi is not None:
            w_hi, w_lo = (ent["hi"], ent["lo"]) if planes is None else planes
            taps = ent["k"] ** 2 if taps is None else taps
            cout, cin = w_hi.shape[1], w_hi.shape[2]
            f = 2 if upsample2x else 1
            oshape = (B, f * H, f * W, cout)
            if out is None:
                out = pool.get(oshape) if want_f32 else None
            oh = ol = None
            if out_split:
                oh, ol = pool.get(oshape, torch.bfloat16), pool.get(oshape, torch.bfloat16)
            kw = {} if not window_origin else dict(window_origin=window_origin)
            if second is not None:
                e2, r_hi, r_lo = second
                kw.update(Cin2=e2["cin"], a2_hi=r_hi, a2_lo=r_lo, w2_hi=e2["hi"], w2_lo=e2["lo"], bias2=e2["bias"])
            part = None
            if stats and out is not None:
                rows = f * f * self._geom(H, W)
                if rows:
                    part = pool.get((B * rows, cout, 2))
            self.be.conv_umma(B=B, H=H, W=W, Cin=cin, Cout=cout, taps=taps, a_hi=a_hi, a_lo=a_lo, w_hi=w_hi,
                              w_lo=w_lo, bias=bias, residual=residual, res_mode=res_mode, out=out, out_hi=oh,
                              out_lo=ol, passes=self.passes, stats_partial=part, upsample2x=upsample2x, **kw)
            if part is not None:
                out._gn = (part, rows)
            return out, oh, ol
        assert second is None and res_mode in (cabi.RES_NONE, cabi.RES_SAME) and not out_split
        cout, k = ent["cout"], ent["k"]
        Ho, Wo = (H + stride - 1) // stride, (W + stride - 1) // stride
        if out is None:
            out = pool.get((B, Ho, Wo, cout))
        self.be.conv_direct(a_f32, ent["f32"], bias, residual, out, cout, k, stride)
        return out, None, None

    def _gn_act(self, pool, x, norm, umma, silu=True, eps=None):
        mean, rstd = self._stats(pool, x, None, eps=eps)
        a_f32 = a_hi = a_lo = None
        if umma:
            a_hi, a_lo = pool.get(x.shape, torch.bfloat16), pool.get(x.shape, torch.bfloat16)
        else:
            a_f32 = pool.get(x.shape)
        self.be.prep(x, None, groups=GN_GROUPS, mean=mean, rstd=rstd, gamma=norm.weight.detach(),
                     beta=norm.bias.detach(), silu=silu, resample=cabi.RESAMPLE_NONE, act_f32=a_f32, act_hi=a_hi,
                     act_lo=a_lo)
        pool.put(mean, rstd)
        return a_f32, a_hi, a_lo

    def _conv_plain(self, pool, ent, x, **kw):
        B, H, W, _ = x.shape
        if "hi" in ent and W >= 4:
            hi, lo = pool.get(x.shape, torch.bfloat16), pool.get(x.shape, torch.bfloat16)
            self.be.prep(x, None, raw_hi=hi, raw_lo=lo)
            out, _, _ = self._conv(pool, ent, a_hi=hi, a_lo=lo, shape=(B, H, W), **kw)
            pool.put(hi, lo)
            return out
        out, _, _ = self._conv(pool, ent, a_f32=x, shape=(B, H, W), **kw)
        return out

    def _head(self, pool, h, norm, ent, out=None):
        B, H, W, _ = h.shape
        if out is not None and "hi_pad" in ent and W >= 4:
            _, a_hi, a_lo = self._gn_act(pool, h, norm, True)
            self.be.conv_umma(B=B, H=H, W=W, Cin=ent["cin"], Cout=64, taps=9, a_hi=a_hi, a_lo=a_lo,
                              w_hi=ent["hi_pad"], w_lo=ent["lo_pad"], bias=ent["bias_pad"], out=out,
                              passes=self.passes, out_nchw_channels=out.shape[1])
            pool.put(a_hi, a_lo, h)
            return out
        a_f32, a_hi, a_lo = self._gn_act(pool, h, norm, "hi" in ent and W >= 4)
        pool.put(h)
        y, _, _ = self._conv(pool, ent, a_f32=a_f32, a_hi=a_hi, a_lo=a_lo, shape=(B, H, W))
        pool.put(a_f32, a_hi, a_lo)
        if out is None:
            return y
        self.be.nhwc_to_nchw(y, out)
        pool.put(y)
        return out

    def _upsample(self, pool, x, ent):
        B, H, W, Cc = x.shape
        if ent is not None and "up_hi" in ent and W >= 4:
            return self._conv_plain(pool, ent, x, planes=(ent["up_hi"], ent["up_lo"]), taps=4, upsample2x=True,
                                    stats=True)
        up = pool.get((B, 2 * H, 2 * W, Cc))
        self.be.prep(x, None, resample=cabi.RESAMPLE_UP2, raw_f32=up)
        if ent is None:
            return up
        out, _, _ = self._conv(pool, ent, a_f32=up, shape=(B, 2 * H, 2 * W))
        pool.put(up)
        return out

    def _avg_pool2(self, pool, x):
        B, H, W, Cc = x.shape
        out = pool.get((B, H // 2, W // 2, Cc))
        self.be.prep(x, None, resample=cabi.RESAMPLE_DOWN2, raw_f32=out)
        return out

    def _skip_residual(self, pool, es, src1, id_mode, r_f32, r_hi, r_lo, shape):
        if es is not None:
            skip, _, _ = self._conv(pool, es, a_f32=r_f32, a_hi=r_hi, a_lo=r_lo, shape=shape)
            return skip, cabi.RES_SAME, skip
        if r_f32 is not None:
            return r_f32, cabi.RES_SAME, None
        return src1, id_mode, None

    def _resblock_flow(self, pool, src1, src2, norm1, norm2, e1, e2, es, resample=cabi.RESAMPLE_NONE, film=None,
                       bias1=None):
        be = self.be
        B, Hs, Ws, c1 = src1.shape
        c2 = 0 if src2 is None else src2.shape[3]
        cin, cout = c1 + c2, e1["cout"]
        H, W = {cabi.RESAMPLE_NONE: (Hs, Ws), cabi.RESAMPLE_UP2: (Hs * 2, Ws * 2),
                cabi.RESAMPLE_DOWN2: (Hs // 2, Ws // 2)}[resample]
        shape, shp = (B, H, W), (B, H, W, cin)
        umma1 = self._umma_ok(cin, cout, W)
        umma2 = self._umma_ok(cout, cout, W)
        fuse_skip = es is not None and umma2 and es["k"] == 1 and cin % 64 == 0
        need_raw_f32 = (es is not None and not fuse_skip) or \
                       (es is None and (src2 is not None or (resample != cabi.RESAMPLE_NONE and not umma2)))
        r_f32 = r_hi = r_lo = None

        mean, rstd = self._stats(pool, src1, src2)
        gkw = dict(groups=GN_GROUPS, mean=mean, rstd=rstd, gamma=norm1.weight.detach(), beta=norm1.bias.detach(),
                   silu=True)
        up_phase = resample == cabi.RESAMPLE_UP2 and umma1 and "up_hi" in e1 and Ws >= 4 and bias1 is None \
            and not need_raw_f32 and not fuse_skip
        if up_phase and self.wino and "up6" in e1 and c1 % 64 == 0:
            u = e1["up6"]
            h1 = convs.wino_conv(be, pool, self._wino_geometry(B, Hs, Ws, 6), src1, src2, cout=cout,
                                 planes=(u["u_hi"], u["u_lo"], u.get("u_inv")), bias=e1["bias"], stats=True, tile=6,
                                 up2_phases=True, **gkw)
            pool.put(mean, rstd)
        elif up_phase:
            a_hi, a_lo = pool.get((B, Hs, Ws, cin), torch.bfloat16), pool.get((B, Hs, Ws, cin), torch.bfloat16)
            be.prep(src1, src2, **gkw, resample=cabi.RESAMPLE_NONE, act_hi=a_hi, act_lo=a_lo)
            pool.put(mean, rstd)
            h1, _, _ = self._conv(pool, e1, a_hi=a_hi, a_lo=a_lo, shape=(B, Hs, Ws), planes=(e1["up_hi"], e1["up_lo"]),
                                  taps=4, upsample2x=True, stats=True)
            pool.put(a_hi, a_lo)
        elif umma1 and not need_raw_f32 and bias1 is None and (
                resample == cabi.RESAMPLE_NONE or (resample == cabi.RESAMPLE_DOWN2 and e1.get("u_tile") == 6
                                                   and not fuse_skip)) and self._wino_ok(e1, B, H, W, c1):
            if fuse_skip:
                r_hi, r_lo = pool.get(shp, torch.bfloat16), pool.get(shp, torch.bfloat16)
            h1 = self._wino_conv(pool, e1, src1, src2, **gkw, raw_hi=r_hi, raw_lo=r_lo,
                                 down2=resample == cabi.RESAMPLE_DOWN2)
            pool.put(mean, rstd)
        else:
            a_f32 = a_hi = a_lo = None
            if umma1:
                a_hi, a_lo = pool.get(shp, torch.bfloat16), pool.get(shp, torch.bfloat16)
            else:
                a_f32 = pool.get(shp)
            if fuse_skip:
                r_hi, r_lo = pool.get(shp, torch.bfloat16), pool.get(shp, torch.bfloat16)
            if need_raw_f32:
                r_f32 = pool.get(shp)
            be.prep(src1, src2, **gkw, resample=resample, act_f32=a_f32, act_hi=a_hi, act_lo=a_lo,
                    raw_f32=r_f32, raw_hi=r_hi, raw_lo=r_lo)
            pool.put(mean, rstd)
            if bias1 is None:
                h1, _, _ = self._conv(pool, e1, a_f32=a_f32, a_hi=a_hi, a_lo=a_lo, shape=shape, stats=True)
            else:
                h1 = pool.get((B, H, W, cout))
                for b in range(B):
                    sl = lambda z: None if z is None else z[b:b + 1]
                    self._conv(pool, e1, a_f32=sl(a_f32), a_hi=sl(a_hi), a_lo=sl(a_lo), shape=(1, H, W),
                               bias=bias1[b], out=h1[b:b + 1])
            pool.put(a_f32, a_hi, a_lo)

        mean, rstd = self._stats(pool, h1, None)
        gkw = dict(groups=GN_GROUPS, mean=mean, rstd=rstd, gamma=norm2.weight.detach(), beta=norm2.bias.detach(),
                   silu=True)
        if film is not None:
            scale, shift = film
            gkw.update(film_scale=scale, film_shift=shift, film_stride=scale.stride(0))
        id_mode = resample_to_res(resample)
        if umma2 and self._wino_ok(e2, B, H, W):
            residual, res_mode, skip_out = self._skip_residual(pool, es, src1, id_mode, r_f32, r_hi, r_lo, shape)
            out = self._wino_conv(pool, e2, h1, None, **gkw, residual=residual, res_mode=res_mode)
            pool.put(mean, rstd, h1)
        else:
            b_f32 = b_hi = b_lo = None
            if umma2:
                b_hi, b_lo = pool.get((B, H, W, cout), torch.bfloat16), pool.get((B, H, W, cout), torch.bfloat16)
            else:
                b_f32 = pool.get((B, H, W, cout))
            be.prep(h1, None, **gkw, resample=cabi.RESAMPLE_NONE, act_f32=b_f32, act_hi=b_hi, act_lo=b_lo)
            pool.put(mean, rstd, h1)
            if fuse_skip:
                second, residual, res_mode, skip_out = (es, r_hi, r_lo), None, cabi.RES_NONE, None
            else:
                second = None
                residual, res_mode, skip_out = self._skip_residual(pool, es, src1, id_mode, r_f32, r_hi, r_lo, shape)
            out, _, _ = self._conv(pool, e2, a_f32=b_f32, a_hi=b_hi, a_lo=b_lo, shape=shape, residual=residual,
                                   res_mode=res_mode, second=second, stats=True)
            pool.put(b_f32, b_hi, b_lo)
        pool.put(r_f32, r_hi, r_lo, skip_out)
        return out

    def _geom(self, H, W):
        key = (H, W)
        r = self._geom_cache.get(key)
        if r is None:
            r = self._geom_cache[key] = self.be.conv_geometry(H, W)[3]
        return r


    def _wino_geometry(self, B, H, W, tile=4):
        key = (B, H, W, tile)
        g = self._wino_geom.get(key)
        if g is None:
            g = self._wino_geom[key] = self.be.wino_geometry(B, H, W, **({} if tile == 4 else dict(tile=tile)))
        return g

    def _wino_ok(self, ent, B, H, W, c1=None):
        if not (self.wino and "u_hi" in ent):
            return False
        tile = ent["u_tile"]
        if tile == 6 and c1 is not None and c1 % 64:
            return False
        return convs.winograd_ok(self._wino_geometry(B, H, W, tile), ent["cin"], ent["cout"], self.wino_min_c,
                                 self.wino_min_tiles, tile)

    def _wino_ready(self, ent, tile=4):
        return self.wino and "hi" in ent and ent["k"] == 3 and convs.wino_channels_ok(ent["cin"], ent["cout"],
                                                                                     self.wino_min_c, tile)

    def _wino_conv(self, pool, ent, src1, src2, *, residual=None, res_mode=cabi.RES_NONE, down2=False, **transform):
        B, H, W, _ = src1.shape
        f = 2 if down2 else 1
        tile = ent["u_tile"]
        return convs.wino_conv(self.be, pool, self._wino_geometry(B, H // f, W // f, tile), src1, src2,
                               cout=ent["cout"], planes=(ent["u_hi"], ent["u_lo"], ent.get("u_inv")), bias=ent["bias"],
                               residual=residual, res_mode=res_mode, stats=True, tile=tile, down2=down2, **transform)


class UNetEngine(KernelExecutor):
    def __init__(self, unet: UNetModel, backend=None, precision: str = "split3"):
        super().__init__(backend, precision)
        self.unet = unet
        self._wkey = None
        self._w = {}
        self._table = None
        self.num_timesteps = 1000
        self.generation = 0

    def _params_key(self):
        return tuple((p.data_ptr(), p._version) for p in self.unet.parameters())

    @staticmethod
    def _ptrs(key):
        return None if key is None else tuple(k[0] for k in key)

    def refresh_weights(self, force=False):
        key = self._params_key()
        if not force and key == self._wkey:
            return
        be, u = self.be, self.unet
        dev = next(u.parameters()).device
        old = self._w or {}
        if self._ptrs(key) != self._ptrs(self._wkey) or not self._w:
            self.generation += 1
        packer = convs.WeightPacker(be, dev, old)
        w = packer.w

        film_w, film_b, off = [], [], 0
        for name, m in u.named_modules():
            if isinstance(m, (nn.Conv2d, nn.Conv1d)):
                packer.conv(name, m.weight, m.bias, padded_head=(name == "out.2"))
            if isinstance(m, ResBlock):
                lin = m.emb_layers[1]
                n = lin.weight.shape[0]
                assert n % 4 == 0
                b = lin.bias.detach()
                if not m.use_scale_shift_norm:
                    b = b + m.in_layers[2].bias.detach()
                film_w.append(lin.weight.detach())
                film_b.append(b)
                w[name + "#film"] = (off, n)
                off += n
        for name, m in u.named_modules():
            if isinstance(m, SpatialTransformer):
                for j, blk in enumerate(m.transformer_blocks):
                    pre = f"{name}.transformer_blocks.{j}"
                    a1, a2 = blk.attn1, blk.attn2
                    packer.conv(pre + ".attn1.qkv", torch.cat([a1.to_q.weight, a1.to_k.weight, a1.to_v.weight], 0), None)
                    packer.conv(pre + ".attn1.to_out.0", a1.to_out[0].weight, a1.to_out[0].bias)
                    packer.conv(pre + ".attn2.to_q", a2.to_q.weight, None)
                    packer.conv(pre + ".attn2.to_kv", torch.cat([a2.to_k.weight, a2.to_v.weight], 0), None)
                    packer.conv(pre + ".attn2.to_out.0", a2.to_out[0].weight, a2.to_out[0].bias)
                    packer.conv(pre + ".ff.net.0.proj", blk.ff.net[0].proj.weight, blk.ff.net[0].proj.bias)
                    packer.conv(pre + ".ff.net.2", blk.ff.net[2].weight, blk.ff.net[2].bias)
        sizes = self._resblock_sizes()
        for name, m in u.named_modules():
            if isinstance(m, ResBlock) and m.use_scale_shift_norm:
                hw = sizes[name]
                tile = convs.wino_tile(hw, hw) if 6 in getattr(be, "wino_tiles", (4,)) else 4
                for cname, conv, direct in ((name + ".in_layers.2", m.in_layers[2], m.up or (m.down and tile != 6)),
                                            (name + ".out_layers.3", m.out_layers[3], False)):
                    if not direct and self._wino_ready(w[cname], tile):
                        packer.winograd(cname, conv.weight, tile)
        for name, m in u.named_modules():
            if isinstance(m, ResBlock) and m.up and m.channels % 64 == 0 and m.out_channels % 64 == 0:
                packer.up_phase(name + ".in_layers.2", m.in_layers[2].weight)
                low = sizes[name] // 2
                if self.wino and 6 in getattr(be, "wino_tiles", (4,)) and convs.wino_tile(low, low) == 6:
                    packer.up_phase_winograd(name + ".in_layers.2", m.in_layers[2].weight)
        if getattr(be, "window_origin", False):
            for name, m in u.named_modules():
                if isinstance(m, Downsample) and m.use_conv and m.channels % 64 == 0 and m.out_channels % 64 == 0:
                    packer.stride2(name + ".op", m.op.weight)
        if old and old.get("film_n") == off and old["film_w"].device == dev:
            w["film_w"], w["film_b"] = old["film_w"], old["film_b"]
            torch.cat(film_w, 0, out=w["film_w"])
            torch.cat(film_b, 0, out=w["film_b"])
        else:
            w["film_w"] = torch.cat(film_w, 0).contiguous()
            w["film_b"] = torch.cat(film_b, 0).contiguous()
        w["film_n"] = off
        self._w = w
        self._wkey = key

    def _resblock_sizes(self):
        u, side, out = self.unet, int(self.unet.image_size), {}
        for prefix, blocks in (("input_blocks", u.input_blocks), ("middle_block", [u.middle_block]),
                               ("output_blocks", u.output_blocks)):
            for i, block in enumerate(blocks):
                for j, layer in enumerate(block):
                    if isinstance(layer, Downsample) or (isinstance(layer, ResBlock) and layer.down):
                        side //= 2
                    elif isinstance(layer, Upsample) or (isinstance(layer, ResBlock) and layer.up):
                        side *= 2
                    if isinstance(layer, ResBlock):
                        out[f"{prefix}.{j}" if prefix == "middle_block" else f"{prefix}.{i}.{j}"] = side
        return out

    def _embedding_table(self, dev):
        want = max(self.num_timesteps, int(getattr(self.unet, "num_timesteps", 0) or 0))
        if self._table is None or self._table.shape[0] < want or self._table.device != dev:
            self.num_timesteps = want
            if self._table is not None:
                self.generation += 1
            tab = timestep_embedding(torch.arange(want), self.unet.model_channels)
            self._table = tab.to(dev).contiguous()
        return self._table

    def _resblock(self, pool, name, m: ResBlock, src1, src2, film):
        w = self._w
        assert src1.shape[3] + (0 if src2 is None else src2.shape[3]) == m.channels
        resample = cabi.RESAMPLE_UP2 if m.up else (cabi.RESAMPLE_DOWN2 if m.down else cabi.RESAMPLE_NONE)
        foff, fn = w[name + "#film"]
        rows = film[:, foff:foff + fn]
        cond = dict(film=rows.chunk(2, dim=1)) if m.use_scale_shift_norm else dict(bias1=rows)
        es = w[name + ".skip_connection"] if isinstance(m.skip_connection, nn.Conv2d) else None
        return self._resblock_flow(pool, src1, src2, m.in_layers[0], m.out_layers[0], w[name + ".in_layers.2"],
                                   w[name + ".out_layers.3"], es, resample, **cond)

    def _attention(self, pool, name, m: AttentionBlock, x):
        be, w = self.be, self._w
        B, H, W, Cc = x.shape
        T = H * W
        eq, ep = w[name + ".qkv"], w[name + ".proj_out"]
        heads = m.num_heads
        hd = Cc // heads
        if hd not in cabi.ATTN_HEAD_DIMS:
            raise NotImplementedError(f"attention head_dim {hd}: the sm_90a kernels support 16/32/64/128")
        umma = self._umma_ok(Cc, Cc, W)
        a_f32, a_hi, a_lo = self._gn_act(pool, x, m.norm, umma, silu=False)
        qkv, q_hi, q_lo = self._conv(pool, eq, a_f32=a_f32, a_hi=a_hi, a_lo=a_lo, shape=(B, H, W),
                                     out_split=umma, want_f32=not umma)
        pool.put(a_f32, a_hi, a_lo)
        o_f32 = o_hi = o_lo = None
        order = 1 if m.new_order else 0
        if umma:
            o_hi, o_lo = pool.get(x.shape, torch.bfloat16), pool.get(x.shape, torch.bfloat16)
            attn = be.attention_tc if hd in cabi.ATTN_TC_HEAD_DIMS else be.attention_split
            attn(q_hi.view(B, T, 3 * Cc), q_lo.view(B, T, 3 * Cc), heads, order,
                 None, o_hi.view(B, T, Cc), o_lo.view(B, T, Cc))
        else:
            o_f32 = pool.get(x.shape)
            be.attention(qkv.view(B, T, 3 * Cc), heads, order, o_f32.view(B, T, Cc), None, None)
        pool.put(qkv, q_hi, q_lo)
        out, _, _ = self._conv(pool, ep, a_f32=o_f32, a_hi=o_hi, a_lo=o_lo, shape=(B, H, W),
                               residual=x, res_mode=cabi.RES_SAME, stats=True)
        pool.put(o_f32, o_hi, o_lo)
        return out

    def _stem(self, pool, ent, x):
        B, H, W, cin = x.shape
        cout = ent["cout"]
        if ent["k"] == 3 and cin <= 16 and cout % 32 == 0 and cout <= 128 and W % 32 == 0 and hasattr(self.be, "conv_stem"):
            out = pool.get((B, H, W, cout))
            part = pool.get((B * H, cout, 2))
            self.be.conv_stem(x, ent["f32"], ent["bias"], out, cout, stats_partial=part)
            out._gn = (part, H)
            return out
        out, _, _ = self._conv(pool, ent, a_f32=x, shape=(B, H, W))
        return out

    def _spatial_transformer(self, pool, name, m: SpatialTransformer, x, ctx):
        be, w = self.be, self._w
        B, H, W, Cc = x.shape
        T, heads, d = H * W, m.n_heads, m.d_head
        inner = heads * d
        if d not in cabi.ATTN_HEAD_DIMS:
            raise NotImplementedError(f"SpatialTransformer head_dim {d}: the sm_90a attention kernels take 16/32/64/128")
        if not (self._umma_ok(Cc, inner, W) and inner % 64 == 0):
            raise NotImplementedError("SpatialTransformer: channel counts must be multiples of 64 (tensor-core GEMMs)")
        bf = torch.bfloat16
        tok = (B, H, W, inner)
        _, a_hi, a_lo = self._gn_act(pool, x, m.norm, True, silu=False, eps=m.norm.eps)
        h, _, _ = self._conv(pool, w[name + ".proj_in"], a_hi=a_hi, a_lo=a_lo, shape=(B, H, W))
        pool.put(a_hi, a_lo)

        def layernorm(ln, src):
            n_hi, n_lo = pool.get(tok, bf), pool.get(tok, bf)
            be.layernorm_split(src, ln.weight.detach(), ln.bias.detach(), ln.eps, out_hi=n_hi, out_lo=n_lo)
            return n_hi, n_lo

        def project_out(ent, o_hi, o_lo, res):
            new, _, _ = self._conv(pool, ent, a_hi=o_hi, a_lo=o_lo, shape=(B, H, W), residual=res, res_mode=cabi.RES_SAME)
            pool.put(o_hi, o_lo, res)
            return new

        for j, blk in enumerate(m.transformer_blocks):
            pre = f"{name}.transformer_blocks.{j}"
            n_hi, n_lo = layernorm(blk.norm1, h)
            _, q_hi, q_lo = self._conv(pool, w[pre + ".attn1.qkv"], a_hi=n_hi, a_lo=n_lo, shape=(B, H, W), out_split=True,
                                       want_f32=False)
            pool.put(n_hi, n_lo)
            o_hi, o_lo = pool.get(tok, bf), pool.get(tok, bf)
            attn = be.attention_tc if d in cabi.ATTN_TC_HEAD_DIMS else be.attention_split
            attn(q_hi.view(B, T, 3 * inner), q_lo.view(B, T, 3 * inner), heads, 1, None, o_hi.view(B, T, inner),
                 o_lo.view(B, T, inner))
            pool.put(q_hi, q_lo)
            h = project_out(w[pre + ".attn1.to_out.0"], o_hi, o_lo, h)
            n_hi, n_lo = layernorm(blk.norm2, h)
            _, q_hi, q_lo = self._conv(pool, w[pre + ".attn2.to_q"], a_hi=n_hi, a_lo=n_lo, shape=(B, H, W), out_split=True,
                                       want_f32=False)
            ekv = w[pre + ".attn2.to_kv"]
            if ctx is None:
                _, kv_hi, kv_lo = self._conv(pool, ekv, a_hi=n_hi, a_lo=n_lo, shape=(B, H, W), out_split=True, want_f32=False)
                Tc = T
            else:
                Bc, Hc, Wc, _ = ctx.shape
                Tc = Hc * Wc
                kv, _, _ = self._conv(pool, ekv, a_f32=ctx, shape=(Bc, Hc, Wc))
                kv_hi, kv_lo = pool.get(kv.shape, bf), pool.get(kv.shape, bf)
                be.prep(kv, None, resample=cabi.RESAMPLE_NONE, raw_hi=kv_hi, raw_lo=kv_lo)
                pool.put(kv)
            pool.put(n_hi, n_lo)
            o_hi, o_lo = pool.get(tok, bf), pool.get(tok, bf)
            be.attention_cross(q_hi.view(B, T, inner), q_lo.view(B, T, inner), kv_hi.view(B, Tc, 2 * inner),
                               kv_lo.view(B, Tc, 2 * inner), heads, None, o_hi.view(B, T, inner), o_lo.view(B, T, inner))
            pool.put(q_hi, q_lo, kv_hi, kv_lo)
            h = project_out(w[pre + ".attn2.to_out.0"], o_hi, o_lo, h)
            if not blk.ff.glu:
                raise NotImplementedError("SpatialTransformer feed-forward without GEGLU")
            n_hi, n_lo = layernorm(blk.norm3, h)
            uu, _, _ = self._conv(pool, w[pre + ".ff.net.0.proj"], a_hi=n_hi, a_lo=n_lo, shape=(B, H, W))
            pool.put(n_hi, n_lo)
            ffi = uu.shape[3] // 2
            g_hi, g_lo = pool.get((B, H, W, ffi), bf), pool.get((B, H, W, ffi), bf)
            be.geglu_split(uu, out_hi=g_hi, out_lo=g_lo)
            pool.put(uu)
            h = project_out(w[pre + ".ff.net.2"], g_hi, g_lo, h)
        r_hi, r_lo = pool.get(tok, bf), pool.get(tok, bf)
        be.prep(h, None, resample=cabi.RESAMPLE_NONE, raw_hi=r_hi, raw_lo=r_lo)
        pool.put(h)
        out, _, _ = self._conv(pool, w[name + ".proj_out"], a_hi=r_hi, a_lo=r_lo, shape=(B, H, W), residual=x,
                               res_mode=cabi.RES_SAME, stats=True)
        pool.put(r_hi, r_lo)
        return out

    def _resample_layer(self, pool, name, m, x):
        if isinstance(m, Upsample):
            return self._upsample(pool, x, self._w[name + ".conv"] if m.use_conv else None)
        if not m.use_conv:
            return self._avg_pool2(pool, x)
        ent = self._w[name + ".op"]
        B, H, W, Cc = x.shape
        if "s2_hi" in ent and H % 2 == 0 and W % 2 == 0 and W // 2 >= 4:
            hi = pool.get((B, H // 2, W // 2, 4 * Cc), torch.bfloat16)
            lo = pool.get((B, H // 2, W // 2, 4 * Cc), torch.bfloat16)
            self.be.s2d_split(x, hi, lo)
            out, _, _ = self._conv(pool, ent, a_hi=hi, a_lo=lo, shape=(B, H // 2, W // 2),
                                   planes=(ent["s2_hi"], ent["s2_lo"]), taps=4, stats=True, window_origin=-1)
            pool.put(hi, lo)
            return out
        out, _, _ = self._conv(pool, ent, a_f32=x, shape=x.shape[:3], stride=2)
        return out

    def _run_block(self, pool, prefix, block: TimestepEmbedSequential, h, skip, film, release_input):
        cur, cur_skip, owned = h, skip, release_input
        for j, layer in enumerate(block):
            name = f"{prefix}.{j}"
            if isinstance(layer, ResBlock):
                new = self._resblock(pool, name, layer, cur, cur_skip, film)
            else:
                assert cur_skip is None, "a concatenated input is only consumed by a ResBlock"
                if isinstance(layer, AttentionBlock):
                    new = self._attention(pool, name, layer, cur)
                elif isinstance(layer, SpatialTransformer):
                    new = self._spatial_transformer(pool, name, layer, cur, self._ctx_nhwc)
                elif isinstance(layer, (Downsample, Upsample)):
                    new = self._resample_layer(pool, name, layer, cur)
                elif isinstance(layer, nn.Conv2d):
                    new = self._stem(pool, self._w[name], cur)
                else:
                    raise NotImplementedError(type(layer).__name__)
            if owned:
                pool.put(cur, cur_skip)
            cur, cur_skip, owned = new, None, True
        return cur

    @torch.no_grad()
    def forward(self, x, timesteps, context=None, assume_fresh_weights=False, out=None):
        u, be = self.unet, self.be
        if not assume_fresh_weights:
            self.refresh_weights()
        w = self._w
        dev = x.device
        x = x.contiguous().float()
        B, Cx, H, W = x.shape
        pool = self._pool(dev, (B, H, W))
        ctx = None
        if u.condition_key != "nocond":
            ctx = context.contiguous().float()
        t = timesteps.to(device=dev, dtype=torch.int64).contiguous()

        mc, ted = u.model_channels, u.model_channels * 4
        temb, e1, emb = pool.get((B, mc)), pool.get((B, ted)), pool.get((B, ted))
        film = pool.get((B, w["film_n"]))
        be.gather_rows(self._embedding_table(dev), t, temb)
        l0, l2 = u.time_embed[0], u.time_embed[2]
        be.linear(temb, l0.weight.detach(), l0.bias.detach(), e1, act_out=True)
        be.linear(e1, l2.weight.detach(), l2.bias.detach(), emb)
        be.linear(emb, w["film_w"], w["film_b"], film, act_in=True)
        pool.put(temb, e1)

        cin0 = Cx + (0 if ctx is None else ctx.shape[1])
        xin = pool.get((B, H, W, cin0))
        be.nchw_to_nhwc_cat(x, ctx, xin)
        self._ctx_nhwc = None
        if getattr(u, "use_spatial_transformer", False) and ctx is not None:
            self._ctx_nhwc = pool.get((B, ctx.shape[2], ctx.shape[3], ctx.shape[1]))
            be.nchw_to_nhwc_cat(ctx, None, self._ctx_nhwc)
        hs = []
        h = xin
        for i, block in enumerate(u.input_blocks):
            h = self._run_block(pool, f"input_blocks.{i}", block, h, None, film, release_input=(i == 0))
            hs.append(h)
        h = self._run_block(pool, "middle_block", u.middle_block, h, None, film, release_input=False)
        for i, block in enumerate(u.output_blocks):
            h = self._run_block(pool, f"output_blocks.{i}", block, h, hs.pop(), film, release_input=True)

        if out is None:
            out = torch.empty((B, u.out_channels, H, W), dtype=torch.float32, device=dev)
        self._head(pool, h, u.out[0], w["out.2"], out)
        pool.put(emb, film, self._ctx_nhwc)
        self._ctx_nhwc = None
        return out
```

include/bbdm_b200.h:

```cpp
#ifndef BBDM_B200_H_
#define BBDM_B200_H_

#include <stdint.h>

#ifdef __cplusplus
extern "C" {
#endif

#define BBDM_ABI_VERSION 7

enum {
  BBDM_OK = 0,
  BBDM_E_INVALID = -1,
  BBDM_E_CUDA = -2,
  BBDM_E_UNSUPPORTED = -3,
  BBDM_E_DEVICE = -4
};

int bbdm_abi_version(void);
const char* bbdm_last_error(void);
int bbdm_device_info(int* sm_count, int* cc_major, int* cc_minor);
int bbdm_check_device_fault(void* stream, unsigned long long* fault_word);


enum { BBDM_OBJ_GRAD = 0, BBDM_OBJ_NOISE = 1, BBDM_OBJ_YSUBX = 2 };

int bbdm_bridge_q_sample(const float* x0, const float* y, const float* noise, const int64_t* t,
                         const float* m_t, const float* variance_t, int num_timesteps,
                         int objective, float* x_t_out, float* objective_out,
                         int B, int64_t n_per_sample, void* stream);

typedef struct {
  float m_t, one_minus_m_t, sqrt_var_t;
  float m_nt, one_minus_m_nt;
  float c_xt;
  float sigma_t;
} BbdmPSampleCoef;

int bbdm_bridge_p_sample(const float* x_t, const float* y, const float* eps, const float* noise,
                         BbdmPSampleCoef coef, int objective, int clip_denoised, int is_last,
                         float* x_out, float* x0_out, int64_t n, void* stream);

int bbdm_bridge_p_sample_dev(const float* x_t, const float* y, const float* eps, const float* noise,
                             const BbdmPSampleCoef* coef_dev, int objective, int clip_denoised,
                             int is_last, float* x_out, float* x0_out, int64_t n, void* stream);


int bbdm_nchw_to_nhwc_cat(const float* x, int c1, const float* ctx, int c2, int B, int H, int W,
                          float* out, void* stream);
int bbdm_nhwc_to_nchw(const float* src, int B, int H, int W, int C, float* out, void* stream);

int bbdm_gather_rows(const float* table, int rows, int width, const int64_t* idx, int B,
                     float* out, void* stream);

int bbdm_linear_f32(const float* x, const float* w, const float* bias, float* out,
                    int B, int K, int N, int act_in, int act_out, void* stream);


#define BBDM_GN_MAX_SLICES 64
int bbdm_gn_stats(const float* src1, int c1, const float* src2, int c2, int B, int H, int W,
                  int groups, float eps, float* mean, float* rstd, double* workspace,
                  void* stream);

enum { BBDM_RESAMPLE_NONE = 0, BBDM_RESAMPLE_UP2 = 1, BBDM_RESAMPLE_DOWN2 = 2 };

typedef struct {
  const float* src1; int c1;
  const float* src2; int c2;
  int B, Hs, Ws;
  int groups;
  const float* mean;
  const float* rstd;
  const float* gamma;
  const float* beta;
  const float* film_scale;
  const float* film_shift;
  int64_t film_stride;
  int silu;
  int resample;
  float* act_f32; void* act_hi; void* act_lo;
  float* raw_f32; void* raw_hi; void* raw_lo;
} BbdmPrepArgs;
int bbdm_prep_operand(const BbdmPrepArgs* a, void* stream);


int bbdm_pack_weight_split(const float* w, int Cout, int Cin, int k, void* w_hi, void* w_lo,
                           void* stream);
int bbdm_pack_weight_split_padded(const float* w, int Cout, int Cin, int k, int Cout_pad,
                                  void* w_hi, void* w_lo, void* stream);
int bbdm_pack_weight_split_taps(const float* w, int Cout, int Cin, int taps, void* w_hi, void* w_lo,
                                void* stream);
int bbdm_pack_weight_split_dgrad(const float* w, int Cout, int Cin, int k, void* w_hi, void* w_lo,
                                 void* stream);

int bbdm_pack_weight_split_both(const float* w, int Cout, int Cin, int k, void* fwd_hi, void* fwd_lo, void* dgrad_hi,
                                void* dgrad_lo, void* stream);
int bbdm_pack_weight_f32(const float* w, int Cout, int Cin, int k, float* out, void* stream);

enum { BBDM_RES_NONE = 0, BBDM_RES_SAME = 1, BBDM_RES_UP2 = 2, BBDM_RES_DOWN2 = 3 };

typedef struct {
  int B, H, W;
  int Cin, Cout, taps;
  const void* a_hi; const void* a_lo;
  const void* w_hi; const void* w_lo;
  const float* bias;
  int Cin2;
  const void* a2_hi; const void* a2_lo;
  const void* w2_hi; const void* w2_lo;
  const float* bias2;
  const float* residual; int res_mode;
  float* out;
  void* out_hi; void* out_lo;
  int passes;
  int out_nchw_channels;
  int upsample2x;
  float* stats_partial;
  int weights_per_image;
  int operand_f16;
  int window_origin;
} BbdmConvArgs;
int bbdm_conv_umma(const BbdmConvArgs* a, void* stream);

int bbdm_conv_umma_geometry(int H, int W, int* TW, int* TH, int* TB, int* rows_per_image);

int bbdm_gn_finalize_partials(const float* part1, int c1, int rows1, const float* part2, int c2,
                              int rows2, int B, int hw, int groups, float eps, float* mean,
                              float* rstd, void* stream);


int bbdm_wino_geometry(int B, int H, int W, int* tiles_h, int* tiles_w, int64_t* tiles_total, int* eligible);

typedef struct {
  const float* src1; int c1;
  const float* src2; int c2;
  int B, H, W;
  int groups;
  const float* mean; const float* rstd; const float* gamma; const float* beta;
  const float* film_scale; const float* film_shift; int64_t film_stride;
  int silu;
  void* v_hi; void* v_lo;
  void* raw_hi; void* raw_lo;
  void* act_hi; void* act_lo;
  int down2;
} BbdmWinoInputArgs;
int bbdm_wino_input(const BbdmWinoInputArgs* a, void* stream);

typedef struct {
  const float* m;
  const float* inv_wscale;
  int B, H, W, Cout;
  const float* bias;
  const float* residual; int res_mode;
  float* out;
  float* stats_partial;
  int up2_phases;
} BbdmWinoOutputArgs;
int bbdm_wino_output(const BbdmWinoOutputArgs* a, void* stream);

int bbdm_wino_pack_weight(const float* w, int Cout, int Cin, int dgrad, void* u_hi, void* u_lo, float* inv_wscale,
                          void* stream);

int bbdm_wino6_geometry(int B, int H, int W, int* tiles_h, int* tiles_w, int64_t* tiles_total, int* eligible);
int bbdm_wino6_input(const BbdmWinoInputArgs* a, void* stream);
int bbdm_wino6_output(const BbdmWinoOutputArgs* a, void* stream);
int bbdm_wino6_pack_weight(const float* w, int Cout, int Cin, int dgrad, void* u_hi, void* u_lo, float* inv_wscale,
                           void* stream);

int bbdm_conv_direct(const float* src, const float* w_packed, const float* bias,
                     const float* residual, float* out, int B, int H, int W, int Cin, int Cout,
                     int k, int stride, void* stream);

int bbdm_conv_stem(const float* src, const float* w_packed, const float* bias, float* out, int B, int H, int W,
                   int Cin, int Cout, float* stats_partial, void* stream);

int bbdm_conv_direct_pad(const float* src, const float* w_packed, const float* bias,
                         const float* residual, float* out, int B, int H, int W, int Cin, int Cout,
                         int k, int stride, int pad_lo, int pad_hi, void* stream);


int bbdm_split_grad(const float* src, int64_t P, int C, void* hi, void* lo, void* hi_t, void* lo_t, int64_t ld_t,
                    float* colsum, float* workspace, void* stream);

int bbdm_conv_wgrad_workspace(int B, int H, int W, int Cin, int Cout, int taps, int* splits,
                              int64_t* floats);

int bbdm_conv_wgrad(const void* g_hi_t, const void* g_lo_t, int64_t ld_g, const void* a_hi, const void* a_lo,
                    int B, int H, int W, int Cin, int Cout, int taps, int window_origin, float* dw,
                    float* workspace, void* stream);

int bbdm_conv_wgrad_direct(const float* dy, const float* x, int B, int H, int W, int Cin, int Cout, int k,
                           float* dw, float* workspace, int64_t workspace_floats, void* stream);

int bbdm_gn_bwd_reduce(const float* x, const float* da, int B, int H, int W, int C, int groups,
                       const float* mean, const float* rstd, const float* gamma, const float* beta,
                       const float* film_scale, const float* film_shift, int64_t film_stride, int silu,
                       float* a12, float* workspace, void* stream);
int bbdm_gn_bwd_apply(const float* x, const float* da, int B, int H, int W, int C, int groups,
                      const float* mean, const float* rstd, const float* gamma, const float* beta,
                      const float* film_scale, const float* film_shift, int64_t film_stride, int silu,
                      const float* s1, const float* s2, float* dx, void* stream);


int bbdm_layernorm_split(const float* x, int64_t rows, int C, const float* gamma, const float* beta, float eps,
                         float* out_f32, void* out_hi, void* out_lo, void* stream);

int bbdm_geglu_split(const float* u, int64_t rows, int N, float* out_f32, void* out_hi, void* out_lo, void* stream);

int bbdm_attention_cross(const void* q_hi, const void* q_lo, const void* kv_hi, const void* kv_lo, int B, int Tq,
                         int Tkv, int C, int heads, float* out_f32, void* out_hi, void* out_lo, void* stream);

int bbdm_layernorm_bwd(const float* x, const float* dy, int64_t rows, int C, const float* gamma, float eps, float* dx,
                       float* dgamma, float* dbeta, float* workspace, void* stream);
int bbdm_geglu_bwd(const float* u, const float* dy, int64_t rows, int N, float* du, void* stream);
int bbdm_attention_cross_bwd(const float* q, const float* kv, const float* out, const float* dout, int B, int Tq, int Tkv,
                             int C, int heads, float* dq, float* dkv, float* lse, float* delta, void* stream);

int bbdm_spatial_rescale(const float* src, int B, int C, int H, int W, int n_stages, const float* w, const float* bias,
                         int Cout, float* out, void* stream);


int bbdm_denorm_to_uint8(const float* images, int B, int C, int H, int W, int to_normal, uint8_t* out, void* stream);

int bbdm_optim_chunk_elems(void);

int bbdm_adam_multi(void* const* params, const void* const* grads, const int64_t* numel, const int64_t* state_off,
                    const int32_t* chunk_tensor, const int32_t* chunk_index, int n_chunks, float* exp_avg,
                    float* exp_avg_sq, double lr, double beta1, double beta2, double eps, double weight_decay, int64_t step,
                    float* ema_shadow, double ema_decay, void* stream);

int bbdm_ema_multi(const void* const* params, const int64_t* numel, const int64_t* state_off,
                   const int32_t* chunk_tensor, const int32_t* chunk_index, int n_chunks, float* shadow, double decay,
                   int with_decay, void* stream);


int bbdm_attention(const float* qkv, int B, int T, int C, int heads, int order,
                   float* out_f32, void* out_hi, void* out_lo, void* stream);

int bbdm_attention_split(const void* qkv_hi, const void* qkv_lo, int B, int T, int C, int heads,
                         int order, float* out_f32, void* out_hi, void* out_lo, void* stream);

int bbdm_attention_tc(const void* qkv_hi, const void* qkv_lo, int B, int T, int C, int heads,
                      int order, float* out_f32, void* out_hi, void* out_lo, void* stream);

int bbdm_attention_bwd(const float* qkv, const float* out, const float* dout, int B, int T, int C, int heads,
                       int order, float* dqkv, float* lse, float* delta, void* stream);

int bbdm_softmax_rows_split(const float* src, int64_t rows, int64_t cols, float scale, void* out_hi,
                            void* out_lo, void* stream);

int bbdm_s2d_split(const float* src, int B, int H, int W, int C, void* out_hi, void* out_lo, void* stream);

int bbdm_vq_nearest(const float* z, const float* codebook, int64_t n_vectors, int n_embed, int dim,
                    float* z_q, long long* indices, void* stream);

#ifdef __cplusplus
}
#endif
#endif
```

Measured before the change: 6.043.

## Feed fp32 activations directly to skip conv, splitting to bf16 in registers

Adds an fp32 A-operand path to the wgmma conv kernel. Activations (optionally a channel concatenation of two sources) are loaded via fp32 TMA maps, split into hi/lo bf16 fragments in registers, and fed to register-sourced wgmma for the three split products. The engine uses this for the skip 1x1 conv in res blocks whose second conv takes the Winograd path, so the prep pass no longer writes separate raw bf16 hi/lo planes. This saves that memory traffic, at the cost of more register and ALU work for in-kernel splitting and serialized wgmma waits.

```diff
diff --git a/bbdm_b200/cabi.py b/bbdm_b200/cabi.py
--- a/bbdm_b200/cabi.py
+++ b/bbdm_b200/cabi.py
@@ -9,7 +9,7 @@
 _HERE = os.path.dirname(os.path.abspath(__file__))
 LIB_PATH = os.environ.get("BBDM_LIB") or os.path.join(_HERE, "libbbdm_b200.so")
 
-ABI_VERSION = 7
+ABI_VERSION = 8
 OBJ = {"grad": 0, "noise": 1, "ysubx": 2}
 RESAMPLE_NONE, RESAMPLE_UP2, RESAMPLE_DOWN2 = 0, 1, 2
 RES_NONE, RES_SAME, RES_UP2, RES_DOWN2 = 0, 1, 2, 3
@@ -67,7 +67,9 @@
                 ("out", C.c_void_p), ("out_hi", C.c_void_p), ("out_lo", C.c_void_p),
                 ("passes", C.c_int), ("out_nchw_channels", C.c_int), ("upsample2x", C.c_int),
                 ("stats_partial", C.c_void_p), ("weights_per_image", C.c_int), ("operand_f16", C.c_int),
-                ("window_origin", C.c_int)]
+                ("window_origin", C.c_int),
+                ("a_f32", C.c_void_p), ("a_f32_cat", C.c_void_p), ("a_c1", C.c_int),
+                ("a2_f32", C.c_void_p), ("a2_f32_cat", C.c_void_p), ("a2_c1", C.c_int)]
 
 
 class WinoInputArgs(C.Structure):
@@ -233,6 +235,7 @@
     name = "sm_90a"
     requires_cuda = True
     wino_tensor_scale = True
+    conv_f32_operand = True
     wino_tiles = (4, 6)
     window_origin = True
 
@@ -342,14 +345,17 @@
         check(self.lib.bbdm_pack_weight_f32(ptr(_req(w)), Cout, Cin, k, ptr(_req(out)), stream()))
         LAUNCHES["n"] += 1
 
-    def conv_umma(self, *, B, H, W, Cin, Cout, taps, a_hi, a_lo, w_hi, w_lo, bias=None, Cin2=0,
+    def conv_umma(self, *, B, H, W, Cin, Cout, taps, a_hi=None, a_lo=None, w_hi, w_lo, bias=None, Cin2=0,
                   a2_hi=None, a2_lo=None, w2_hi=None, w2_lo=None, bias2=None, residual=None,
                   res_mode=RES_NONE, out=None, out_hi=None, out_lo=None, passes=3, out_nchw_channels=0,
-                  stats_partial=None, upsample2x=False, weights_per_image=False, operand_f16=False, window_origin=0):
+                  stats_partial=None, upsample2x=False, weights_per_image=False, operand_f16=False, window_origin=0,
+                  a_f32=None, a_f32_cat=None, a2_f32=None, a2_f32_cat=None):
         a = ConvArgs(B, H, W, Cin, Cout, taps, ptr(a_hi), ptr(a_lo), ptr(w_hi), ptr(w_lo), ptr(bias),
                      Cin2, ptr(a2_hi), ptr(a2_lo), ptr(w2_hi), ptr(w2_lo), ptr(bias2),
                      ptr(residual), res_mode, ptr(out), ptr(out_hi), ptr(out_lo), passes, out_nchw_channels,
-                     int(upsample2x), ptr(stats_partial), int(weights_per_image), int(operand_f16), int(window_origin))
+                     int(upsample2x), ptr(stats_partial), int(weights_per_image), int(operand_f16), int(window_origin),
+                     ptr(a_f32), ptr(None if a_f32_cat is None else _req(a_f32_cat)), 0 if a_f32 is None else _req(a_f32).shape[-1],
+                     ptr(a2_f32), ptr(None if a2_f32_cat is None else _req(a2_f32_cat)), 0 if a2_f32 is None else _req(a2_f32).shape[-1])
         check(self.lib.bbdm_conv_umma(C.byref(a), stream()))
         LAUNCHES["n"] += 1
 
diff --git a/bbdm_b200/csrc/conv_umma.cu b/bbdm_b200/csrc/conv_umma.cu
--- a/bbdm_b200/csrc/conv_umma.cu
+++ b/bbdm_b200/csrc/conv_umma.cu
@@ -21,6 +21,7 @@
   int origin;
   int w_per_image;
   int kb_per_chunk;
+  int a_c1, a2_c1;
   const float* bias; const float* bias2;
   const float* residual; int res_mode;
   float* out; __nv_bfloat16* out_hi; __nv_bfloat16* out_lo;
@@ -39,6 +40,53 @@
   static constexpr int STAGES3 = (SMEM_BUDGET / STAGE3) > 6 ? 6 : (SMEM_BUDGET / STAGE3);
   static constexpr int STAGES1 = (SMEM_BUDGET / STAGE1) > 8 ? 8 : (SMEM_BUDGET / STAGE1);
 };
+
+template <int BN>
+__device__ __forceinline__ void conv_mma_rs(float* d, const uint32_t* a, uint64_t db) {
+  if (BN == 128) wgmma_rs_n128_bf16<0>(d, a, db, 1u); else wgmma_rs_n64_bf16<0>(d, a, db, 1u);
+}
+
+template <int A_BYTES>
+__device__ __forceinline__ void af32_fragment(uint32_t sbase, int k, uint32_t* hi, uint32_t* lo) {
+  int t = threadIdx.x;
+  asm volatile("" : "+r"(t));
+  const int lane = t & 31, q = lane & 3, sw = lane >> 2;
+  const uint32_t box = sbase + (uint32_t)(t >> 5 << 4 | sw) * 128 + (k >> 1) * A_BYTES;
+#pragma unroll
+  for (int j = 0; j < 2; ++j) {
+    const uint32_t col = (uint32_t)((((4 * (k & 1) + (q >> 1) + 2 * j) ^ sw) << 4) + (q & 1) * 8);
+#pragma unroll
+    for (int ri = 0; ri < 2; ++ri) {
+      float x, y;
+      asm volatile("ld.shared.v2.f32 {%0, %1}, [%2];" : "=f"(x), "=f"(y) : "r"(box + ri * 8 * 128 + col) : "memory");
+      split2x(x, y, hi[2 * j + ri], lo[2 * j + ri]);
+    }
+  }
+}
+
+template <int BN, uint32_t A_BYTES, bool CHAIN>
+__device__ __forceinline__ void af32_kblock(float* acc, uint32_t sbase, uint64_t db_hi, uint64_t db_lo,
+                                            uint32_t (*f_hi)[4], uint32_t (*f_lo)[4], bool first) {
+#pragma unroll
+  for (int k = 0; k < UM_BK / 16; ++k) {
+    const uint64_t ko = (uint64_t)(k * 32 >> 4);
+    uint32_t* hi = f_hi[k & 1];
+    uint32_t* lo = f_lo[k & 1];
+    af32_fragment<A_BYTES>(sbase, k, hi, lo);
+    wgmma_fence();
+    conv_mma_rs<BN>(acc, lo, db_hi + ko);
+    conv_mma_rs<BN>(acc, hi, db_lo + ko);
+    conv_mma_rs<BN>(acc, hi, db_hi + ko);
+    wgmma_commit();
+    if (CHAIN || k + 1 < UM_BK / 16) {
+      reg_fence_u<4>(hi); reg_fence_u<4>(lo);
+      wgmma_wait<1>();
+      if (k > 0 || (CHAIN && !first)) { reg_fence_u<4>(f_hi[(k + 1) & 1]); reg_fence_u<4>(f_lo[(k + 1) & 1]); }
+    } else {
+      wgmma_wait<0>();
+    }
+  }
+}
 
 template <int BN, bool F16>
 __device__ __forceinline__ void conv_mma(float* d, uint64_t da, uint64_t db) {
@@ -205,7 +253,7 @@
     if (s >= s_begin && s < s_end) epi_slice<BN>(p, racc, e, s, warp, lane, stats_s);
 }
 
-template <int BN, int PASSES, bool F16>
+template <int BN, int PASSES, bool F16, bool AF32>
 __global__ void __launch_bounds__(UM_THREADS, 1)
 conv_umma_kernel(const __grid_constant__ CUtensorMap map_a_hi, const __grid_constant__ CUtensorMap map_a_lo,
                  const __grid_constant__ CUtensorMap map_w_hi, const __grid_constant__ CUtensorMap map_w_lo,
@@ -220,6 +268,7 @@
   constexpr uint32_t OFF_WLO = OFF_WHI + Cfg::W_BYTES;
   constexpr int NR = BN / 2;
   static_assert(STAGES >= 2, "need at least a double buffer");
+  static_assert(!AF32 || (PASSES == 3 && !F16), "fp32 A operand: split bf16, three products");
 
   extern __shared__ uint8_t smem_raw[];
   __shared__ __align__(8) uint64_t bars[2 * 8];
@@ -273,14 +322,30 @@
             } else if (p.taps == 9) { dy = tap / 3 - 1; dx = tap % 3 - 1; }
             else if (p.taps == 4) { dy = (tap >> 1) + p.origin; dx = (tap & 1) + p.origin; }
             else if (p.w_per_image) wtap = tb;
-            tma_load_4d(sbase, &map_a_hi, full, cb * UM_BK, w0 + dx, h0 + dy, b0);
-            if (PASSES == 3) tma_load_4d(sbase + OFF_ALO, &map_a_lo, full, cb * UM_BK, w0 + dx, h0 + dy, b0);
+            if (AF32) {
+              const bool second = cb * UM_BK >= p.a_c1;
+              const CUtensorMap* m = second ? &map_a_lo : &map_a_hi;
+              const int c = cb * UM_BK - (second ? p.a_c1 : 0);
+              tma_load_4d(sbase, m, full, c, w0 + dx, h0 + dy, b0);
+              tma_load_4d(sbase + OFF_ALO, m, full, c + UM_BK / 2, w0 + dx, h0 + dy, b0);
+            } else {
+              tma_load_4d(sbase, &map_a_hi, full, cb * UM_BK, w0 + dx, h0 + dy, b0);
+              if (PASSES == 3) tma_load_4d(sbase + OFF_ALO, &map_a_lo, full, cb * UM_BK, w0 + dx, h0 + dy, b0);
+            }
             tma_load_3d(sbase + OFF_WHI, &map_w_hi, full, cb * UM_BK, n0, wtap);
             if (PASSES == 3) tma_load_3d(sbase + OFF_WLO, &map_w_lo, full, cb * UM_BK, n0, wtap);
           } else {
             const int cb = kb - p.K1;
-            tma_load_4d(sbase, &map_a2_hi, full, cb * UM_BK, w0, h0, b0);
-            if (PASSES == 3) tma_load_4d(sbase + OFF_ALO, &map_a2_lo, full, cb * UM_BK, w0, h0, b0);
+            if (AF32) {
+              const bool second = cb * UM_BK >= p.a2_c1;
+              const CUtensorMap* m = second ? &map_a2_lo : &map_a2_hi;
+              const int c = cb * UM_BK - (second ? p.a2_c1 : 0);
+              tma_load_4d(sbase, m, full, c, w0, h0, b0);
+              tma_load_4d(sbase + OFF_ALO, m, full, c + UM_BK / 2, w0, h0, b0);
+            } else {
+              tma_load_4d(sbase, &map_a2_hi, full, cb * UM_BK, w0, h0, b0);
+              if (PASSES == 3) tma_load_4d(sbase + OFF_ALO, &map_a2_lo, full, cb * UM_BK, w0, h0, b0);
+            }
             tma_load_3d(sbase + OFF_WHI, &map_w2_hi, full, cb * UM_BK, n0, 0);
             if (PASSES == 3) tma_load_3d(sbase + OFF_WLO, &map_w2_lo, full, cb * UM_BK, n0, 0);
           }
@@ -307,6 +372,18 @@
 #pragma unroll
       for (int j = 0; j < NR; ++j) acc[j] = 0.f;
       int prev = -1;
+      if (AF32 && !pending) {
+        uint32_t f_hi[2][4], f_lo[2][4];
+        for (int kb = kb0; kb < kb1; ++kb) {
+          mbar_wait(bar_full + 8 * stage, phase_bit, abort_flag, p.fault, 0xF0000000ull | (unsigned)kb);
+          const uint32_t sbase = tiles_base + stage * STAGE_BYTES;
+          af32_kblock<BN, Cfg::A_BYTES, true>(acc, sbase, make_sw128_desc(sbase + OFF_WHI),
+                                              make_sw128_desc(sbase + OFF_WLO), f_hi, f_lo, kb == kb0);
+          if (prev >= 0 && lane == 0) mbar_arrive(bar_empty + 8 * prev);
+          prev = stage;
+          if (++stage == STAGES) { stage = 0; phase_bit ^= 1; }
+        }
+      } else
       for (int kb = kb0; kb < kb1; ++kb) {
         mbar_wait(bar_full + 8 * stage, phase_bit, abort_flag, p.fault, 0xF0000000ull | (unsigned)kb);
         const uint32_t sbase = tiles_base + stage * STAGE_BYTES;
@@ -314,18 +391,23 @@
         const uint64_t da_lo = make_sw128_desc(sbase + OFF_ALO + a_off);
         const uint64_t db_hi = make_sw128_desc(sbase + OFF_WHI);
         const uint64_t db_lo = make_sw128_desc(sbase + OFF_WLO);
-        wgmma_fence();
-#pragma unroll
-        for (int k = 0; k < UM_BK / 16; ++k) {
-          const uint64_t ko = (uint64_t)(k * 32 >> 4);
-          if (PASSES == 3) {
-            conv_mma<BN, F16>(acc, da_lo + ko, db_hi + ko);
-            conv_mma<BN, F16>(acc, da_hi + ko, db_lo + ko);
+        if (AF32) {
+          uint32_t f_hi[2][4], f_lo[2][4];
+          af32_kblock<BN, Cfg::A_BYTES, false>(acc, sbase, db_hi, db_lo, f_hi, f_lo, true);
+        } else {
+          wgmma_fence();
+#pragma unroll
+          for (int k = 0; k < UM_BK / 16; ++k) {
+            const uint64_t ko = (uint64_t)(k * 32 >> 4);
+            if (PASSES == 3) {
+              conv_mma<BN, F16>(acc, da_lo + ko, db_hi + ko);
+              conv_mma<BN, F16>(acc, da_hi + ko, db_lo + ko);
+            }
+            conv_mma<BN, F16>(acc, da_hi + ko, db_hi + ko);
           }
-          conv_mma<BN, F16>(acc, da_hi + ko, db_hi + ko);
+          wgmma_commit();
+          wgmma_wait<1>();
         }
-        wgmma_commit();
-        wgmma_wait<1>();
         if (prev >= 0 && lane == 0) mbar_arrive(bar_empty + 8 * prev);
         prev = stage;
         if (++stage == STAGES) { stage = 0; phase_bit ^= 1; }
@@ -361,14 +443,17 @@
 }
 
 static int make_act_map(CUtensorMap* m, const void* ptr, int B, int H, int W, int C, int TW, int TH, int TB,
-                        bool f16) {
+                        bool f16, bool f32 = false) {
   EncodeTiledFn enc = get_encode();
   BBDM_REQUIRE(enc != nullptr, "cuTensorMapEncodeTiled entry point not available");
+  const int es_bytes = f32 ? 4 : 2;
   cuuint64_t dims[4] = {(cuuint64_t)C, (cuuint64_t)W, (cuuint64_t)H, (cuuint64_t)B};
-  cuuint64_t strides[3] = {(cuuint64_t)C * 2, (cuuint64_t)W * C * 2, (cuuint64_t)H * W * C * 2};
-  cuuint32_t box[4] = {(cuuint32_t)UM_BK, (cuuint32_t)TW, (cuuint32_t)TH, (cuuint32_t)TB};
+  cuuint64_t strides[3] = {(cuuint64_t)C * es_bytes, (cuuint64_t)W * C * es_bytes, (cuuint64_t)H * W * C * es_bytes};
+  cuuint32_t box[4] = {(cuuint32_t)(128 / es_bytes), (cuuint32_t)TW, (cuuint32_t)TH, (cuuint32_t)TB};
   cuuint32_t es[4] = {1, 1, 1, 1};
-  CUresult r = enc(m, f16 ? CU_TENSOR_MAP_DATA_TYPE_FLOAT16 : CU_TENSOR_MAP_DATA_TYPE_BFLOAT16, 4, const_cast<void*>(ptr), dims, strides, box, es,
+  const CUtensorMapDataType dt = f32 ? CU_TENSOR_MAP_DATA_TYPE_FLOAT32
+                                     : (f16 ? CU_TENSOR_MAP_DATA_TYPE_FLOAT16 : CU_TENSOR_MAP_DATA_TYPE_BFLOAT16);
+  CUresult r = enc(m, dt, 4, const_cast<void*>(ptr), dims, strides, box, es,
                    CU_TENSOR_MAP_INTERLEAVE_NONE, CU_TENSOR_MAP_SWIZZLE_128B, CU_TENSOR_MAP_L2_PROMOTION_L2_256B,
                    CU_TENSOR_MAP_FLOAT_OOB_FILL_NONE);
   BBDM_REQUIRE(r == CUDA_SUCCESS, "cuTensorMapEncodeTiled(activation) failed: %d (B=%d H=%d W=%d C=%d box=%dx%dx%d)",
@@ -394,7 +479,7 @@
 static int pow2_floor(int x) { int p = 1; while (p * 2 <= x) p *= 2; return p; }
 static int pow2_ceil(int x) { int p = 1; while (p < x) p *= 2; return p; }
 
-template <int BN, int PASSES, bool F16>
+template <int BN, int PASSES, bool F16, bool AF32 = false>
 static int launch_conv(const CUtensorMap* maps, const ConvParams& p, int grid, cudaStream_t s) {
   using Cfg = UmmaCfg<BN>;
   constexpr int STAGES = PASSES == 3 ? Cfg::STAGES3 : Cfg::STAGES1;
@@ -402,10 +487,10 @@
   const size_t smem = (size_t)STAGES * STAGE_BYTES + 1024;
   static DeviceOnce configured;
   if (configured.need()) {
-    BBDM_CUDA_CHECK(cudaFuncSetAttribute(conv_umma_kernel<BN, PASSES, F16>, cudaFuncAttributeMaxDynamicSharedMemorySize, (int)smem));
+    BBDM_CUDA_CHECK(cudaFuncSetAttribute(conv_umma_kernel<BN, PASSES, F16, AF32>, cudaFuncAttributeMaxDynamicSharedMemorySize, (int)smem));
     configured.mark();
   }
-  conv_umma_kernel<BN, PASSES, F16><<<grid, UM_THREADS, smem, s>>>(maps[0], maps[1], maps[2], maps[3], maps[4], maps[5],
+  conv_umma_kernel<BN, PASSES, F16, AF32><<<grid, UM_THREADS, smem, s>>>(maps[0], maps[1], maps[2], maps[3], maps[4], maps[5],
                                                                   maps[6], maps[7], p);
   BBDM_LAUNCH_CHECK();
   return BBDM_OK;
@@ -442,8 +527,27 @@
   BBDM_REQUIRE(a->Cout > 0 && a->Cout % 64 == 0, "conv_umma: Cout %% 64 != 0 (Cout=%d)", a->Cout);
   BBDM_REQUIRE(a->Cin2 >= 0 && a->Cin2 % 64 == 0, "conv_umma: Cin2 %% 64 != 0 (Cin2=%d)", a->Cin2);
   BBDM_REQUIRE(a->passes == 1 || a->passes == 3, "conv_umma: passes must be 1 or 3");
-  BBDM_REQUIRE(a->a_hi && a->w_hi && (a->passes == 1 || (a->a_lo && a->w_lo)), "conv_umma: missing operand plane");
-  if (a->Cin2) BBDM_REQUIRE(a->a2_hi && a->w2_hi && (a->passes == 1 || (a->a2_lo && a->w2_lo)), "conv_umma: missing 1x1 operand plane");
+  const bool af32 = a->a_f32 != nullptr;
+  if (af32) {
+    BBDM_REQUIRE(a->passes == 3 && !a->operand_f16 && !a->weights_per_image && !a->upsample2x && !a->a_hi && !a->a_lo,
+                 "conv_umma: the fp32 A operand needs passes 3, bf16 weight planes, no upsample2x / weights_per_image, "
+                 "and no A planes");
+    BBDM_REQUIRE(a->a_c1 > 0 && a->a_c1 % 64 == 0 && a->a_c1 <= a->Cin && (a->a_c1 == a->Cin) == (a->a_f32_cat == nullptr),
+                 "conv_umma: a_c1 must be a multiple of 64, Cin without a_f32_cat and less with it (a_c1=%d Cin=%d)",
+                 a->a_c1, a->Cin);
+    BBDM_REQUIRE(a->w_hi && a->w_lo, "conv_umma: missing weight plane");
+    if (a->Cin2) {
+      BBDM_REQUIRE(a->a2_f32 && !a->a2_hi && !a->a2_lo && a->w2_hi && a->w2_lo, "conv_umma: fp32 A needs an fp32 A2");
+      BBDM_REQUIRE(a->a2_c1 > 0 && a->a2_c1 % 64 == 0 && a->a2_c1 <= a->Cin2 &&
+                   (a->a2_c1 == a->Cin2) == (a->a2_f32_cat == nullptr),
+                   "conv_umma: a2_c1 must be a multiple of 64, Cin2 without a2_f32_cat and less with it (a2_c1=%d Cin2=%d)",
+                   a->a2_c1, a->Cin2);
+    }
+  } else {
+    BBDM_REQUIRE(!a->a_f32_cat && !a->a2_f32 && !a->a2_f32_cat, "conv_umma: fp32 A2 / second source without a_f32");
+    BBDM_REQUIRE(a->a_hi && a->w_hi && (a->passes == 1 || (a->a_lo && a->w_lo)), "conv_umma: missing operand plane");
+    if (a->Cin2) BBDM_REQUIRE(a->a2_hi && a->w2_hi && (a->passes == 1 || (a->a2_lo && a->w2_lo)), "conv_umma: missing 1x1 operand plane");
+  }
   BBDM_REQUIRE(a->out || (a->out_hi && a->out_lo), "conv_umma: no output");
   BBDM_REQUIRE((a->out_hi == nullptr) == (a->out_lo == nullptr), "conv_umma: out hi/lo must come in pairs");
   BBDM_REQUIRE(a->res_mode >= 0 && a->res_mode <= 3 && (a->res_mode == 0 || a->residual), "conv_umma: bad residual");
@@ -476,6 +580,8 @@
   p.up2 = a->upsample2x ? 1 : 0;
   p.origin = a->window_origin;
   p.w_per_image = wpi ? 1 : 0;
+  p.a_c1 = af32 ? a->a_c1 : 0;
+  p.a2_c1 = af32 ? a->a2_c1 : 0;
   static int wino_chunk = -1;
   if (wino_chunk < 0) { const char* e = getenv("BBDM_WINO_CHUNK"); wino_chunk = (e && atoi(e) > 0) ? atoi(e) : 0; }
   const int wchunk = wino_chunk ? wino_chunk : (a->Cin >= 512 ? 4 : 2);
@@ -495,14 +601,34 @@
                "conv_umma: stats_partial needs a tile inside one image (H*W >= 128) and NHWC output");
   CUtensorMap maps[8];
   int rc;
-  if ((rc = make_act_map(&maps[0], a->a_hi, a->B, a->H, a->W, a->Cin, p.TW, p.TH, p.TB, f16))) return rc;
-  if ((rc = make_act_map(&maps[1], a->passes == 3 ? a->a_lo : a->a_hi, a->B, a->H, a->W, a->Cin, p.TW, p.TH, p.TB, f16))) return rc;
+  if (af32) {
+    const int cr = a->Cin - a->a_c1;
+    if ((rc = make_act_map(&maps[0], a->a_f32, a->B, a->H, a->W, a->a_c1, p.TW, p.TH, p.TB, false, true))) return rc;
+    if (cr) {
+      if ((rc = make_act_map(&maps[1], a->a_f32_cat, a->B, a->H, a->W, cr, p.TW, p.TH, p.TB, false, true))) return rc;
+    } else {
+      maps[1] = maps[0];
+    }
+  } else {
+    if ((rc = make_act_map(&maps[0], a->a_hi, a->B, a->H, a->W, a->Cin, p.TW, p.TH, p.TB, f16))) return rc;
+    if ((rc = make_act_map(&maps[1], a->passes == 3 ? a->a_lo : a->a_hi, a->B, a->H, a->W, a->Cin, p.TW, p.TH, p.TB, f16))) return rc;
+  }
   const int wtaps = a->upsample2x ? 16 : (wpi ? a->B : a->taps);
   if ((rc = make_w_map(&maps[2], a->w_hi, wtaps, a->Cout, a->Cin, BN, f16))) return rc;
   if ((rc = make_w_map(&maps[3], a->passes == 3 ? a->w_lo : a->w_hi, wtaps, a->Cout, a->Cin, BN, f16))) return rc;
   if (a->Cin2) {
-    if ((rc = make_act_map(&maps[4], a->a2_hi, a->B, a->H, a->W, a->Cin2, p.TW, p.TH, p.TB, f16))) return rc;
-    if ((rc = make_act_map(&maps[5], a->passes == 3 ? a->a2_lo : a->a2_hi, a->B, a->H, a->W, a->Cin2, p.TW, p.TH, p.TB, f16))) return rc;
+    if (af32) {
+      const int cr = a->Cin2 - a->a2_c1;
+      if ((rc = make_act_map(&maps[4], a->a2_f32, a->B, a->H, a->W, a->a2_c1, p.TW, p.TH, p.TB, false, true))) return rc;
+      if (cr) {
+        if ((rc = make_act_map(&maps[5], a->a2_f32_cat, a->B, a->H, a->W, cr, p.TW, p.TH, p.TB, false, true))) return rc;
+      } else {
+        maps[5] = maps[4];
+      }
+    } else {
+      if ((rc = make_act_map(&maps[4], a->a2_hi, a->B, a->H, a->W, a->Cin2, p.TW, p.TH, p.TB, f16))) return rc;
+      if ((rc = make_act_map(&maps[5], a->passes == 3 ? a->a2_lo : a->a2_hi, a->B, a->H, a->W, a->Cin2, p.TW, p.TH, p.TB, f16))) return rc;
+    }
     if ((rc = make_w_map(&maps[6], a->w2_hi, 1, a->Cout, a->Cin2, BN, f16))) return rc;
     if ((rc = make_w_map(&maps[7], a->passes == 3 ? a->w2_lo : a->w2_hi, 1, a->Cout, a->Cin2, BN, f16))) return rc;
   } else {
@@ -513,6 +639,7 @@
   const int grid = (int)(total < num_sms() ? total : num_sms());
   cudaStream_t s = (cudaStream_t)stream;
   const bool p3 = a->passes == 3;
+  if (af32) return BN == 128 ? launch_conv<128, 3, false, true>(maps, p, grid, s) : launch_conv<64, 3, false, true>(maps, p, grid, s);
   if (BN == 128) {
     if (f16) return p3 ? launch_conv<128, 3, true>(maps, p, grid, s) : launch_conv<128, 1, true>(maps, p, grid, s);
     return p3 ? launch_conv<128, 3, false>(maps, p, grid, s) : launch_conv<128, 1, false>(maps, p, grid, s);
diff --git a/bbdm_b200/csrc/tc_common.cuh b/bbdm_b200/csrc/tc_common.cuh
--- a/bbdm_b200/csrc/tc_common.cuh
+++ b/bbdm_b200/csrc/tc_common.cuh
@@ -74,6 +74,11 @@
 #pragma unroll
   for (int i = 0; i < R; ++i) asm volatile("" : "+f"(d[i])::"memory");
 }
+template <int R>
+__device__ __forceinline__ void reg_fence_u(uint32_t* a) {
+#pragma unroll
+  for (int i = 0; i < R; ++i) asm volatile("" : "+r"(a[i])::"memory");
+}
 
 __device__ __forceinline__ uint64_t make_sw128_desc(uint32_t saddr, uint32_t lbo = 16) {
   uint64_t d = 0;
@@ -130,6 +135,16 @@
       : "r"(a[0]), "r"(a[1]), "r"(a[2]), "r"(a[3]), "l"(db), "r"(scale_d), "n"(TB));
 }
 
+template <int TB>
+__device__ __forceinline__ void wgmma_rs_n128_bf16(float* d, const uint32_t* a, uint64_t db, uint32_t scale_d) {
+  asm volatile(
+      "{\n\t.reg .pred p;\n\tsetp.ne.b32 p, %69, 0;\n\t"
+      "wgmma.mma_async.sync.aligned.m64n128k16.f32.bf16.bf16 "
+      "{%0, %1, %2, %3, %4, %5, %6, %7, %8, %9, %10, %11, %12, %13, %14, %15, %16, %17, %18, %19, %20, %21, %22, %23, %24, %25, %26, %27, %28, %29, %30, %31, %32, %33, %34, %35, %36, %37, %38, %39, %40, %41, %42, %43, %44, %45, %46, %47, %48, %49, %50, %51, %52, %53, %54, %55, %56, %57, %58, %59, %60, %61, %62, %63}, {%64, %65, %66, %67}, %68, p, 1, 1, %70;\n\t}"
+      : "+f"(d[0]), "+f"(d[1]), "+f"(d[2]), "+f"(d[3]), "+f"(d[4]), "+f"(d[5]), "+f"(d[6]), "+f"(d[7]), "+f"(d[8]), "+f"(d[9]), "+f"(d[10]), "+f"(d[11]), "+f"(d[12]), "+f"(d[13]), "+f"(d[14]), "+f"(d[15]), "+f"(d[16]), "+f"(d[17]), "+f"(d[18]), "+f"(d[19]), "+f"(d[20]), "+f"(d[21]), "+f"(d[22]), "+f"(d[23]), "+f"(d[24]), "+f"(d[25]), "+f"(d[26]), "+f"(d[27]), "+f"(d[28]), "+f"(d[29]), "+f"(d[30]), "+f"(d[31]), "+f"(d[32]), "+f"(d[33]), "+f"(d[34]), "+f"(d[35]), "+f"(d[36]), "+f"(d[37]), "+f"(d[38]), "+f"(d[39]), "+f"(d[40]), "+f"(d[41]), "+f"(d[42]), "+f"(d[43]), "+f"(d[44]), "+f"(d[45]), "+f"(d[46]), "+f"(d[47]), "+f"(d[48]), "+f"(d[49]), "+f"(d[50]), "+f"(d[51]), "+f"(d[52]), "+f"(d[53]), "+f"(d[54]), "+f"(d[55]), "+f"(d[56]), "+f"(d[57]), "+f"(d[58]), "+f"(d[59]), "+f"(d[60]), "+f"(d[61]), "+f"(d[62]), "+f"(d[63])
+      : "r"(a[0]), "r"(a[1]), "r"(a[2]), "r"(a[3]), "l"(db), "r"(scale_d), "n"(TB));
+}
+
 template <int N>
 __device__ __forceinline__ void setmaxnreg_inc() { asm volatile("setmaxnreg.inc.sync.aligned.u32 %0;" ::"n"(N)); }
 template <int N>
diff --git a/bbdm_b200/engine.py b/bbdm_b200/engine.py
--- a/bbdm_b200/engine.py
+++ b/bbdm_b200/engine.py
@@ -98,10 +98,10 @@
 
     def _conv(self, pool, ent, *, a_f32=None, a_hi=None, a_lo=None, shape, bias=None, residual=None,
               res_mode=cabi.RES_NONE, second=None, out_split=False, want_f32=True, stride=1, out=None,
-              stats=False, planes=None, taps=None, upsample2x=False, window_origin=0):
+              stats=False, planes=None, taps=None, upsample2x=False, window_origin=0, a_cat=None):
         B, H, W = shape
         bias = ent["bias"] if bias is None else bias
-        if a_hi is not None:
+        if a_hi is not None or a_cat is not None:
             w_hi, w_lo = (ent["hi"], ent["lo"]) if planes is None else planes
             taps = ent["k"] ** 2 if taps is None else taps
             cout, cin = w_hi.shape[1], w_hi.shape[2]
@@ -113,6 +113,8 @@
             if out_split:
                 oh, ol = pool.get(oshape, torch.bfloat16), pool.get(oshape, torch.bfloat16)
             kw = {} if not window_origin else dict(window_origin=window_origin)
+            if a_cat is not None:
+                kw.update(a_f32=a_cat[0], a_f32_cat=a_cat[1])
             if second is not None:
                 e2, r_hi, r_lo = second
                 kw.update(Cin2=e2["cin"], a2_hi=r_hi, a2_lo=r_lo, w2_hi=e2["hi"], w2_lo=e2["lo"], bias2=e2["bias"])
@@ -197,9 +199,9 @@
         self.be.prep(x, None, resample=cabi.RESAMPLE_DOWN2, raw_f32=out)
         return out
 
-    def _skip_residual(self, pool, es, src1, id_mode, r_f32, r_hi, r_lo, shape):
+    def _skip_residual(self, pool, es, src1, id_mode, r_f32, r_hi, r_lo, r_cat, shape):
         if es is not None:
-            skip, _, _ = self._conv(pool, es, a_f32=r_f32, a_hi=r_hi, a_lo=r_lo, shape=shape)
+            skip, _, _ = self._conv(pool, es, a_f32=r_f32, a_hi=r_hi, a_lo=r_lo, a_cat=r_cat, shape=shape)
             return skip, cabi.RES_SAME, skip
         if r_f32 is not None:
             return r_f32, cabi.RES_SAME, None
@@ -220,6 +222,10 @@
         need_raw_f32 = (es is not None and not fuse_skip) or \
                        (es is None and (src2 is not None or (resample != cabi.RESAMPLE_NONE and not umma2)))
         r_f32 = r_hi = r_lo = None
+        wino2 = umma2 and self._wino_ok(e2, B, H, W)
+        r_cat = (src1, src2) if (fuse_skip and wino2 and resample == cabi.RESAMPLE_NONE and c1 % 64 == 0 and
+                                 getattr(type(be), "conv_f32_operand", False)) else None
+        raw_planes = fuse_skip and r_cat is None
 
         mean, rstd = self._stats(pool, src1, src2)
         gkw = dict(groups=GN_GROUPS, mean=mean, rstd=rstd, gamma=norm1.weight.detach(), beta=norm1.bias.detach(),
@@ -242,7 +248,7 @@
         elif umma1 and not need_raw_f32 and bias1 is None and (
                 resample == cabi.RESAMPLE_NONE or (resample == cabi.RESAMPLE_DOWN2 and e1.get("u_tile") == 6
                                                    and not fuse_skip)) and self._wino_ok(e1, B, H, W, c1):
-            if fuse_skip:
+            if raw_planes:
                 r_hi, r_lo = pool.get(shp, torch.bfloat16), pool.get(shp, torch.bfloat16)
             h1 = self._wino_conv(pool, e1, src1, src2, **gkw, raw_hi=r_hi, raw_lo=r_lo,
                                  down2=resample == cabi.RESAMPLE_DOWN2)
@@ -253,7 +259,7 @@
                 a_hi, a_lo = pool.get(shp, torch.bfloat16), pool.get(shp, torch.bfloat16)
             else:
                 a_f32 = pool.get(shp)
-            if fuse_skip:
+            if raw_planes:
                 r_hi, r_lo = pool.get(shp, torch.bfloat16), pool.get(shp, torch.bfloat16)
             if need_raw_f32:
                 r_f32 = pool.get(shp)
@@ -277,8 +283,9 @@
             scale, shift = film
             gkw.update(film_scale=scale, film_shift=shift, film_stride=scale.stride(0))
         id_mode = resample_to_res(resample)
-        if umma2 and self._wino_ok(e2, B, H, W):
-            residual, res_mode, skip_out = self._skip_residual(pool, es, src1, id_mode, r_f32, r_hi, r_lo, shape)
+        if wino2:
+            residual, res_mode, skip_out = self._skip_residual(pool, es, src1, id_mode, r_f32, r_hi, r_lo, r_cat,
+                                                               shape)
             out = self._wino_conv(pool, e2, h1, None, **gkw, residual=residual, res_mode=res_mode)
             pool.put(mean, rstd, h1)
         else:
@@ -293,7 +300,8 @@
                 second, residual, res_mode, skip_out = (es, r_hi, r_lo), None, cabi.RES_NONE, None
             else:
                 second = None
-                residual, res_mode, skip_out = self._skip_residual(pool, es, src1, id_mode, r_f32, r_hi, r_lo, shape)
+                residual, res_mode, skip_out = self._skip_residual(pool, es, src1, id_mode, r_f32, r_hi, r_lo, None,
+                                                                   shape)
             out, _, _ = self._conv(pool, e2, a_f32=b_f32, a_hi=b_hi, a_lo=b_lo, shape=shape, residual=residual,
                                    res_mode=res_mode, second=second, stats=True)
             pool.put(b_f32, b_hi, b_lo)
diff --git a/include/bbdm_b200.h b/include/bbdm_b200.h
--- a/include/bbdm_b200.h
+++ b/include/bbdm_b200.h
@@ -7,7 +7,7 @@
 extern "C" {
 #endif
 
-#define BBDM_ABI_VERSION 7
+#define BBDM_ABI_VERSION 8
 
 enum {
   BBDM_OK = 0,
@@ -119,6 +119,8 @@
   int weights_per_image;
   int operand_f16;
   int window_origin;
+  const float* a_f32; const float* a_f32_cat; int a_c1;
+  const float* a2_f32; const float* a2_f32_cat; int a2_c1;
 } BbdmConvArgs;
 int bbdm_conv_umma(const BbdmConvArgs* a, void* stream);
 
```

New measurement: 6.061, median of 6. Within noise of the previous version (+0.3%).
